# Tyler-Sch/pyruhvro

Measured on NVIDIA H100. Metric: avro_to_arrow_records_per_sec, higher is better.
Workload: dtype u8

## Files before the change

### include/ruhvro_b200.h

```cpp
#ifndef RUHVRO_B200_H
#define RUHVRO_B200_H

#include <stddef.h>
#include <stdint.h>

#ifdef __cplusplus
extern "C" {
#endif

struct ArrowSchema;
struct ArrowArray;
struct ArrowDeviceArray;

typedef struct rv_schema rv_schema;
typedef struct rv_result rv_result;
typedef struct rv_encoded rv_encoded;

typedef enum rv_status {
    RV_OK = 0,
    RV_ERR_EOF = 1,
    RV_ERR_VARINT = 2,
    RV_ERR_BOOL = 3,
    RV_ERR_NEG_LEN = 4,
    RV_ERR_BRANCH = 5,
    RV_ERR_ENUM = 6,
    RV_ERR_SCHEMA = 7,
    RV_ERR_OVERFLOW = 8,
    RV_ERR_INVALID = 9,
    RV_ERR_CUDA = 10,
    RV_ERR_VALUE = 11,
    RV_ERR_FRAME = 12
} rv_status;


rv_status rv_schema_parse(const char* json, size_t len, rv_schema** out);
rv_schema* rv_schema_retain(rv_schema* s);
void rv_schema_release(rv_schema* s);

int rv_schema_is_supported(const rv_schema* s);

rv_status rv_schema_export_arrow(const rv_schema* s, struct ArrowSchema* out);

rv_status rv_schema_project(const rv_schema* s, const char* const* columns, int64_t n_columns, rv_schema** out);


rv_status rv_decode_host(const rv_schema* s, const uint8_t* data, const int64_t* offsets, int64_t n,
                         int64_t num_chunks, rv_result** out);

rv_status rv_decode_device(const rv_schema* s, const uint8_t* d_data, const int64_t* d_offsets, int64_t n,
                           int64_t num_chunks, void* cuda_stream, rv_result** out);

typedef struct rv_framing {
    int32_t header_bytes;
    int32_t check_magic;
    int64_t schema_id;
} rv_framing;
rv_status rv_decode_host_framed(const rv_schema* s, const uint8_t* data, const int64_t* offsets, int64_t n,
                                int64_t num_chunks, const rv_framing* framing, rv_result** out);
rv_status rv_decode_device_framed(const rv_schema* s, const uint8_t* d_data, const int64_t* d_offsets, int64_t n,
                                  int64_t num_chunks, const rv_framing* framing, void* cuda_stream, rv_result** out);

rv_status rv_decode_ocf_host(const uint8_t* file, int64_t len, int64_t num_chunks, rv_schema** schema_out, rv_result** out);

rv_status rv_decode_ocf_host_projected(const uint8_t* file, int64_t len, int64_t num_chunks, const char* const* columns,
                                       int64_t n_columns, rv_schema** schema_out, rv_result** out);

rv_status rv_result_to_host(rv_result* r);

int64_t rv_result_num_batches(const rv_result* r);
int64_t rv_result_num_rows(const rv_result* r, int64_t batch);
int64_t rv_result_arrow_bytes(const rv_result* r);

int64_t rv_result_buffer_bytes(const rv_result* r);

rv_status rv_result_export(rv_result* r, int64_t batch, struct ArrowArray* out_array, struct ArrowSchema* out_schema);
rv_status rv_result_export_device(rv_result* r, int64_t batch, struct ArrowDeviceArray* out_array, struct ArrowSchema* out_schema);

void rv_result_free(rv_result* r);

rv_status rv_encode_host(const rv_schema* s, struct ArrowArray* batch, struct ArrowSchema* batch_schema, int64_t num_chunks, rv_encoded** out);
int64_t rv_encoded_num_chunks(const rv_encoded* r);
rv_status rv_encoded_export(rv_encoded* r, int64_t chunk, struct ArrowArray* out_array, struct ArrowSchema* out_schema);
void rv_encoded_free(rv_encoded* r);
int rv_last_encode_timings(float* out_ms, int cap);

typedef struct rv_gather rv_gather;
int64_t rv_gather_meta_len(const rv_schema* s);
rv_status rv_result_gather_meta(const rv_result* r, int64_t batch, int64_t* out, int64_t cap);
rv_status rv_gather_plan(const rv_schema* s, const int64_t* metas , int world, rv_gather** out);
int rv_gather_num_groups(const rv_gather* g);
int rv_gather_group_of_rank(const rv_gather* g, int rank);
rv_status rv_gather_group_info(const rv_gather* g, int group, int64_t* out5);
rv_status rv_gather_alloc(rv_gather* g, int group, void* cuda_stream, void** out_dev_ptr);
rv_status rv_gather_push(rv_gather* g, int group, int rank, rv_result* mine, int64_t batch, void* dst_base, void* cuda_stream);
rv_status rv_gather_finish(rv_gather* g, int group, rv_result** out);
void rv_gather_free(rv_gather* g);
rv_status rv_ipc_export(void* dev_ptr, uint8_t* handle64);
rv_status rv_ipc_open(const uint8_t* handle64, void** out_dev_ptr);
rv_status rv_ipc_close(void* dev_ptr);

rv_status rv_dev_rebase_i32(int32_t* d_dst, const int32_t* d_src, int64_t n, int32_t add, void* cuda_stream);
rv_status rv_dev_concat_bits(uint32_t* d_dst_words, int64_t dst_bit, const uint32_t* d_src_words, int64_t nbits, void* cuda_stream);


void* rv_host_alloc(size_t bytes);
void rv_host_free(void* p);

int rv_last_timings(float* out_ms, int cap);
int rv_last_launch_count(void);
int rv_last_passes(void);
void rv_schema_forget_stats(const rv_schema* s);

const char* rv_last_walker(void);
const char* rv_schema_jit_status(const rv_schema* s);
long long rv_last_slow_tiles(void);
void rv_set_jit_enabled(int enabled);

int64_t rv_schema_walker_source(const rv_schema* s, char* buf, size_t cap);

rv_status rv_schema_precompile(const rv_schema* s, const char* arch);

const char* rv_last_error(void);
const char* rv_version(void);

#ifdef __cplusplus
}
#endif

#endif
```

### pyruhvro_b200/__init__.py

```python
from __future__ import annotations

import ctypes
import os
import threading
from typing import List

import pyarrow as pa

from . import _build

__all__ = [
    "deserialize_array", "deserialize_array_threaded", "deserialize_array_threaded_spawn",
    "serialize_record_batch", "serialize_record_batch_spawn", "lib", "Schema", "decode_packed", "deserialize_arrow_array",
    "deserialize_confluent", "deserialize_ocf",
]

_HERE = os.path.dirname(os.path.abspath(__file__))


class _ArrowSchema(ctypes.Structure):
    _fields_ = [("format", ctypes.c_char_p), ("name", ctypes.c_char_p), ("metadata", ctypes.c_char_p),
                ("flags", ctypes.c_int64), ("n_children", ctypes.c_int64), ("children", ctypes.c_void_p),
                ("dictionary", ctypes.c_void_p), ("release", ctypes.c_void_p), ("private_data", ctypes.c_void_p)]


class _ArrowArray(ctypes.Structure):
    _fields_ = [("length", ctypes.c_int64), ("null_count", ctypes.c_int64), ("offset", ctypes.c_int64),
                ("n_buffers", ctypes.c_int64), ("n_children", ctypes.c_int64), ("buffers", ctypes.c_void_p),
                ("children", ctypes.c_void_p), ("dictionary", ctypes.c_void_p), ("release", ctypes.c_void_p),
                ("private_data", ctypes.c_void_p)]


def _load():
    path = os.path.join(_HERE, "libruhvro_b200.so")
    if os.environ.get("RV_LIB_PATH"):
        return _bind(ctypes.CDLL(os.environ["RV_LIB_PATH"]))
    try:
        _build.build_all()
    except Exception:
        if not os.path.exists(path):
            raise
    return _bind(ctypes.CDLL(path))


def _bind(L):
    vp, i64, cp = ctypes.c_void_p, ctypes.c_int64, ctypes.c_char_p
    L.rv_schema_parse.argtypes = [cp, ctypes.c_size_t, ctypes.POINTER(vp)]
    L.rv_schema_retain.restype = vp
    L.rv_schema_retain.argtypes = [vp]
    L.rv_schema_release.argtypes = [vp]
    L.rv_schema_release.restype = None
    L.rv_schema_is_supported.argtypes = [vp]
    L.rv_schema_export_arrow.argtypes = [vp, vp]
    L.rv_decode_host.argtypes = [vp, vp, vp, i64, i64, ctypes.POINTER(vp)]
    L.rv_decode_device.argtypes = [vp, vp, vp, i64, i64, vp, ctypes.POINTER(vp)]
    L.rv_decode_host_framed.argtypes = [vp, vp, vp, i64, i64, vp, ctypes.POINTER(vp)]
    L.rv_decode_device_framed.argtypes = [vp, vp, vp, i64, i64, vp, vp, ctypes.POINTER(vp)]
    L.rv_decode_ocf_host.argtypes = [vp, i64, i64, ctypes.POINTER(vp), ctypes.POINTER(vp)]
    L.rv_decode_ocf_host_projected.argtypes = [vp, i64, i64, vp, i64, ctypes.POINTER(vp), ctypes.POINTER(vp)]
    L.rv_schema_project.argtypes = [vp, vp, i64, ctypes.POINTER(vp)]
    L.rv_result_to_host.argtypes = [vp]
    L.rv_result_num_batches.restype = i64
    L.rv_result_num_batches.argtypes = [vp]
    L.rv_result_num_rows.restype = i64
    L.rv_result_num_rows.argtypes = [vp, i64]
    L.rv_result_arrow_bytes.restype = i64
    L.rv_result_arrow_bytes.argtypes = [vp]
    L.rv_result_buffer_bytes.restype = i64
    L.rv_result_buffer_bytes.argtypes = [vp]
    L.rv_result_export.argtypes = [vp, i64, vp, vp]
    L.rv_result_export_device.argtypes = [vp, i64, vp, vp]
    L.rv_result_free.argtypes = [vp]
    L.rv_result_free.restype = None
    L.rv_encode_host.argtypes = [vp, vp, vp, i64, ctypes.POINTER(vp)]
    L.rv_encoded_num_chunks.restype = i64
    L.rv_encoded_num_chunks.argtypes = [vp]
    L.rv_encoded_export.argtypes = [vp, i64, vp, vp]
    L.rv_encoded_free.argtypes = [vp]
    L.rv_encoded_free.restype = None
    L.rv_host_alloc.restype = vp
    L.rv_host_alloc.argtypes = [ctypes.c_size_t]
    L.rv_host_free.argtypes = [vp]
    L.rv_host_free.restype = None
    L.rv_last_timings.argtypes = [ctypes.POINTER(ctypes.c_float), ctypes.c_int]
    L.rv_last_launch_count.restype = ctypes.c_int
    L.rv_last_slow_tiles.restype = ctypes.c_longlong
    L.rv_last_passes.restype = ctypes.c_int
    L.rv_schema_forget_stats.argtypes = [vp]
    L.rv_schema_forget_stats.restype = None
    L.rv_last_walker.restype = cp
    L.rv_set_jit_enabled.argtypes = [ctypes.c_int]
    L.rv_set_jit_enabled.restype = None
    L.rv_schema_walker_source.restype = i64
    L.rv_schema_walker_source.argtypes = [vp, cp, ctypes.c_size_t]
    L.rv_schema_precompile.argtypes = [vp, cp]
    L.rv_last_error.restype = cp
    L.rv_version.restype = cp
    return L


lib = _load()


def last_walker() -> str:
    return (lib.rv_last_walker() or b"").decode()


def set_jit_enabled(enabled: int) -> None:
    lib.rv_set_jit_enabled(int(enabled))


def _last_error() -> str:
    return (lib.rv_last_error() or b"").decode("utf-8", "replace")


def _check(status: int):
    if status != 0:
        raise ValueError(_last_error())


class Schema:

    def __init__(self, schema_json: str):
        raw = schema_json.encode("utf-8")
        h = ctypes.c_void_p()
        _check(lib.rv_schema_parse(raw, len(raw), ctypes.byref(h)))
        self.handle = h.value
        self._arrow = None

    def __del__(self):
        h, self.handle = getattr(self, "handle", None), None
        if h:
            lib.rv_schema_release(h)

    @classmethod
    def _adopt(cls, handle: int) -> "Schema":
        s = cls.__new__(cls)
        s.handle, s._arrow = handle, None
        return s

    def project(self, columns) -> "Schema":
        names, keep = _column_names(columns)
        h = ctypes.c_void_p()
        _check(lib.rv_schema_project(self.handle, names, len(keep), ctypes.byref(h)))
        return Schema._adopt(h.value)

    @property
    def is_supported(self) -> bool:
        return bool(lib.rv_schema_is_supported(self.handle))

    def precompile(self, arch: str = "sm_90a") -> None:
        _check(lib.rv_schema_precompile(self.handle, arch.encode()))

    @property
    def walker_source(self) -> str:
        n = lib.rv_schema_walker_source(self.handle, None, 0)
        if n < 0:
            raise ValueError("schema has no decode plan")
        buf = ctypes.create_string_buffer(n + 1)
        lib.rv_schema_walker_source(self.handle, buf, n + 1)
        return buf.value.decode()

    @property
    def arrow_schema(self) -> pa.Schema:
        if self._arrow is None:
            cs = _ArrowSchema()
            _check(lib.rv_schema_export_arrow(self.handle, ctypes.addressof(cs)))
            self._arrow = pa.Schema._import_from_c(ctypes.addressof(cs))
        return self._arrow


def _column_names(columns):
    if isinstance(columns, (str, bytes)):
        raise TypeError("argument 'columns': expected a list of field names, not a single string")
    keep = []
    for c in columns:
        if not isinstance(c, str):
            raise TypeError("argument 'columns': field names must be str")
        keep.append(c.encode("utf-8"))
    arr = (ctypes.c_char_p * max(len(keep), 1))(*keep)
    return arr, keep


_schema_cache = {}
_schema_lock = threading.Lock()


def _get_or_parse_schema(schema: str, columns=None) -> Schema:
    if not isinstance(schema, str):
        raise TypeError("argument 'schema': expected str")
    if columns is not None:
        if isinstance(columns, (str, bytes)):
            raise TypeError("argument 'columns': expected a list of field names, not a single string")
        columns = tuple(columns)
    key = (schema, columns)
    with _schema_lock:
        s = _schema_cache.get(key)
    if s is not None:
        return s
    parsed = Schema(schema) if columns is None else _get_or_parse_schema(schema).project(columns)
    with _schema_lock:
        return _schema_cache.setdefault(key, parsed)


def _export_batches(result_handle: int, schema: Schema) -> List[pa.RecordBatch]:
    try:
        arrow_schema = schema.arrow_schema
        out = []
        for i in range(lib.rv_result_num_batches(result_handle)):
            arr = _ArrowArray()
            _check(lib.rv_result_export(result_handle, i, ctypes.addressof(arr), None))
            out.append(pa.RecordBatch._import_from_c(ctypes.addressof(arr), arrow_schema))
        return out
    finally:
        lib.rv_result_free(result_handle)


_native_mod = None


def _ext():
    global _native_mod
    if _native_mod is None:
        import importlib
        _native_mod = importlib.import_module(__name__ + "._native")
    return _native_mod


class Framing(ctypes.Structure):
    _fields_ = [("header_bytes", ctypes.c_int32), ("check_magic", ctypes.c_int32), ("schema_id", ctypes.c_int64)]


def _decode_list(records, schema: str, num_chunks: int, framing=None, columns=None) -> List[pa.RecordBatch]:
    if not isinstance(records, list):
        raise TypeError("argument 'list': expected a list of bytes")
    s = _get_or_parse_schema(schema, columns)
    if framing is None:
        handle = _ext().decode_list(s.handle, records, int(num_chunks))
    else:
        handle = _ext().decode_list(s.handle, records, int(num_chunks), *framing)
    return _export_batches(handle, s)




def deserialize_ocf(data, num_chunks=1, *, columns=None) -> List[pa.RecordBatch]:
    import numpy as np
    if num_chunks < 0:
        raise OverflowError("can't convert negative int to unsigned")
    buf = np.frombuffer(data, dtype=np.uint8)
    sh, h = ctypes.c_void_p(), ctypes.c_void_p()
    if columns is None:
        _check(lib.rv_decode_ocf_host(buf.ctypes.data if buf.size else None, buf.size, int(num_chunks), ctypes.byref(sh), ctypes.byref(h)))
    else:
        names, keep = _column_names(columns)
        _check(lib.rv_decode_ocf_host_projected(buf.ctypes.data if buf.size else None, buf.size, int(num_chunks), names, len(keep),
                                                ctypes.byref(sh), ctypes.byref(h)))
    return _export_batches(h.value, Schema._adopt(sh.value))


def deserialize_confluent(list, schema, num_chunks=1, schema_id=None, *, columns=None):
    if num_chunks < 0:
        raise OverflowError("can't convert negative int to unsigned")
    return _decode_list(list, schema, num_chunks, framing=(5, 1, -1 if schema_id is None else int(schema_id)), columns=columns)


def deserialize_array(list, schema, *, columns=None):
    return _decode_list(list, schema, 1, columns=columns)[0]


def deserialize_array_threaded(list, schema, num_chunks, *, columns=None):
    if num_chunks < 0:
        raise OverflowError("can't convert negative int to unsigned")
    return _decode_list(list, schema, num_chunks, columns=columns)


def deserialize_array_threaded_spawn(list, schema, num_chunks, *, columns=None):
    return deserialize_array_threaded(list, schema, num_chunks, columns=columns)


def decode_packed(data, offsets, n: int, schema: str, num_chunks: int = 1, framing: "Framing | None" = None, *,
                  columns=None) -> List[pa.RecordBatch]:
    import numpy as np
    s = _get_or_parse_schema(schema, columns)
    data = np.ascontiguousarray(data, dtype=np.uint8)
    offsets = np.ascontiguousarray(offsets, dtype=np.int64)
    h = ctypes.c_void_p()
    _check(lib.rv_decode_host_framed(s.handle, data.ctypes.data if data.size else None, offsets.ctypes.data, n, num_chunks,
                                     ctypes.byref(framing) if framing is not None else None, ctypes.byref(h)))
    return _export_batches(h.value, s)


def _packed_view(arr):
    import numpy as np
    if isinstance(arr, pa.ChunkedArray):
        arr = arr.combine_chunks() if arr.num_chunks != 1 else arr.chunk(0)
    t = arr.type
    if pa.types.is_large_binary(t) or pa.types.is_large_string(t):
        odt = np.int64
    elif pa.types.is_binary(t) or pa.types.is_string(t):
        odt = np.int32
    else:
        raise TypeError(f"expected a (Large)Binary / (Large)String array of Avro datums, got {t}")
    if arr.null_count:
        raise ValueError("the datum array contains nulls")
    n = len(arr)
    bufs = arr.buffers()
    if n == 0 or bufs[1] is None:
        return np.zeros(0, dtype=np.uint8), np.zeros(1, dtype=np.int64), 0
    off = np.frombuffer(bufs[1], dtype=odt)[arr.offset: arr.offset + n + 1]
    data = np.frombuffer(bufs[2], dtype=np.uint8) if bufs[2] is not None else np.zeros(0, dtype=np.uint8)
    return data, off.astype(np.int64, copy=False), n


def deserialize_arrow_array(array, schema, num_chunks=1, *, columns=None):
    if num_chunks < 0:
        raise OverflowError("can't convert negative int to unsigned")
    data, off, n = _packed_view(array)
    return decode_packed(data, off, n, schema, int(num_chunks), columns=columns)


def serialize_record_batch(data, schema, num_chunks):
    if not isinstance(data, pa.RecordBatch):
        raise TypeError("argument 'data': expected a pyarrow.RecordBatch")
    if num_chunks < 0:
        raise OverflowError("can't convert negative int to unsigned")
    s = _get_or_parse_schema(schema)
    c_arr, c_sch = _ArrowArray(), _ArrowSchema()
    data._export_to_c(ctypes.addressof(c_arr), ctypes.addressof(c_sch))
    h = ctypes.c_void_p()
    _check(lib.rv_encode_host(s.handle, ctypes.addressof(c_arr), ctypes.addressof(c_sch), int(num_chunks), ctypes.byref(h)))
    try:
        out = []
        for i in range(lib.rv_encoded_num_chunks(h)):
            a, sc = _ArrowArray(), _ArrowSchema()
            _check(lib.rv_encoded_export(h, i, ctypes.addressof(a), ctypes.addressof(sc)))
            out.append(pa.Array._import_from_c(ctypes.addressof(a), ctypes.addressof(sc)))
        return out
    finally:
        lib.rv_encoded_free(h)


def serialize_record_batch_spawn(data, schema, num_chunks):
    return serialize_record_batch(data, schema, num_chunks)
```

### pyruhvro_b200/csrc/dev_kernels.cuh

```cuda
#pragma once
#include "dev_core.cuh"

namespace rv {

struct Tile {
    int chunk;
    int local_tile;
    int lin;
    int64_t r0;
    int nrec;
    int64_t chunk_len;
};

__device__ __forceinline__ Tile tile_of(const DecodeParams& p, int id) {
    Tile t;
    int j = 0, local = id;
    if (p.k > 1) {
        const int body = p.k * p.tiles_per_chunk;
        if (id < body) {
            local = int(__fdividef(float(id), float(p.k)));
            while (local > 0 && local * p.k > id) --local;
            while ((local + 1) * p.k <= id) ++local;
            j = id - local * p.k;
        } else {
            j = p.k - 1;
            local = p.tiles_per_chunk + (id - body);
        }
    }
    t.chunk = j;
    t.local_tile = local;
    t.lin = j * p.tiles_per_chunk + local;
    const int64_t cs = int64_t(j) * p.chunk_rows;
    const int64_t ce = (j == p.k - 1) ? p.n : cs + p.chunk_rows;
    t.chunk_len = ce - cs;
    t.r0 = cs + int64_t(t.local_tile) * kBlock;
    const int64_t left = ce - t.r0;
    t.nrec = left < kBlock ? int(left) : kBlock;
    return t;
}

struct TileWindow {
    bool staged;
    bool tma;
    int64_t t0, t1;
    uint32_t mis;
    int64_t o0, o1;
    int64_t f0, f1;
};

__device__ __forceinline__ void l2_prefetch_line(const void* p) { asm volatile("prefetch.global.L2 [%0];" ::"l"(p)); }
__device__ __forceinline__ void l2_prefetch_bulk(const void* p, uint32_t bytes) {
    asm volatile("cp.async.bulk.prefetch.L2.global [%0], %1;" ::"l"(p), "r"(bytes) : "memory");
}
constexpr int kPrefetchLane = 32;

__device__ __forceinline__ uint32_t smem_addr(const void* p) { return uint32_t(__cvta_generic_to_shared(p)); }
__device__ __forceinline__ void mbar_init(uint32_t mbar, uint32_t arrivals) {
    asm volatile("mbarrier.init.shared::cta.b64 [%0], %1;" ::"r"(mbar), "r"(arrivals) : "memory");
    asm volatile("fence.mbarrier_init.release.cluster;" ::: "memory");
}
__device__ __forceinline__ void bulk_load(uint32_t dst, const void* src, uint32_t bytes, uint32_t mbar) {
    asm volatile("mbarrier.arrive.expect_tx.shared::cta.b64 _, [%0], %1;" ::"r"(mbar), "r"(bytes) : "memory");
    asm volatile("cp.async.bulk.shared::cluster.global.mbarrier::complete_tx::bytes [%0], [%1], %2, [%3];"
                 ::"r"(dst), "l"(src), "r"(bytes), "r"(mbar) : "memory");
}
__device__ __forceinline__ void mbar_wait(uint32_t mbar, uint32_t parity) {
    asm volatile(
        "{\n"
        ".reg .pred P1;\n"
        "RV_WAIT:\n"
        "mbarrier.try_wait.parity.shared::cta.b64 P1, [%0], %1;\n"
        "@P1 bra RV_DONE;\n"
        "bra RV_WAIT;\n"
        "RV_DONE:\n"
        "}" ::"r"(mbar), "r"(parity) : "memory");
}

constexpr unsigned long long kStAgg = 1ull << 62;
constexpr unsigned long long kStPrefix = 2ull << 62;
constexpr unsigned long long kStMask = (1ull << 62) - 1ull;

__device__ __forceinline__ unsigned long long ld_state(const unsigned long long* p) {
    unsigned long long v;
    asm volatile("ld.relaxed.gpu.global.u64 %0, [%1];" : "=l"(v) : "l"(p) : "memory");
    return v;
}
__device__ __forceinline__ void st_state(unsigned long long* p, unsigned long long v) {
    asm volatile("st.relaxed.gpu.global.u64 [%0], %1;" ::"l"(p), "l"(v) : "memory");
}

__device__ __forceinline__ unsigned long long look_back(const unsigned long long* st, const int tile, const int first) {
    const int lane = threadIdx.x & 31;
    unsigned long long excl = 0;
    int t = tile - 1;
    for (;;) {
        const int mine = t - lane;
        const bool real = mine >= first;
        unsigned long long v;
        do { v = real ? ld_state(st + mine) : kStPrefix; } while (__any_sync(0xFFFFFFFFu, (v >> 62) == 0ull));
        const unsigned has = __ballot_sync(0xFFFFFFFFu, (v >> 62) == 2ull);
        const int pl = has ? __ffs(int(has)) - 1 : 32;
        unsigned long long c = lane <= pl ? (v & kStMask) : 0ull;
#pragma unroll
        for (int d = 16; d; d >>= 1) c += __shfl_xor_sync(0xFFFFFFFFu, c, d);
        excl += c;
        if (has) break;
        t -= 32;
    }
    return excl;
}

template <class W>
__device__ __forceinline__ TileWindow stage_in(const DecodeParams& p, const Tile& t, const int tile_id, const SmemMap& m) {
    const int tid = threadIdx.x;
    if (tid == 0) mbar_init(smem_addr(rv_smem + m.mbar), 1);
    if (p.n_nodes) {
        uint4* dn = reinterpret_cast<uint4*>(rv_smem + m.nodes);
        for (int i = tid; i < p.n_nodes * 2; i += kBlock) dn[i] = __ldg(reinterpret_cast<const uint4*>(p.nodes) + i);
    }
    if (p.bufs) {
        void** sp = reinterpret_cast<void**>(rv_smem + m.ptrs);
        void* const* gp = p.bufs + size_t(t.chunk) * p.n_slots;
        for (int i = tid; i < p.n_slots; i += kBlock) sp[i] = gp[i];
    }
    if constexpr (!W::kRegCursors) {
        uint32_t* cur = reinterpret_cast<uint32_t*>(rv_smem + m.cur);
        for (int s = 0; s < p.n_streams; ++s) cur[s * kBlock + tid] = 0;
    }
    if (tid == 0) *reinterpret_cast<uint32_t*>(rv_smem + m.flags) = 0u;
    TileWindow w;
    w.t0 = __ldg(p.offsets + t.r0);
    w.t1 = __ldg(p.offsets + t.r0 + t.nrec);
    w.o0 = w.o1 = 0;
    if (tid < t.nrec) {
        w.o0 = __ldg(p.offsets + t.r0 + tid);
        w.o1 = __ldg(p.offsets + t.r0 + tid + 1);
    }
    w.f0 = w.f1 = -1;
    const int64_t ft = int64_t(tile_id) + p.prefetch_dist;
    if (p.prefetch_dist > 0 && ft < p.n_tiles) {
        const Tile f = tile_of(p, int(ft));
        if (tid < 17 && f.r0 + 16 * tid <= p.n) l2_prefetch_line(p.offsets + f.r0 + 16 * tid);
        if (tid == kPrefetchLane) {
            w.f0 = __ldg(p.offsets + f.r0);
            w.f1 = __ldg(p.offsets + f.r0 + f.nrec);
        }
    }
    const int64_t span = w.t1 - w.t0;
    w.mis = uint32_t(reinterpret_cast<uintptr_t>(p.data + w.t0) & 15u);
    w.staged = span >= 0 && uint64_t(span) + w.mis <= uint64_t(p.smem_data_cap);
    w.tma = false;
    if (w.staged) {
        const uint4* g = reinterpret_cast<const uint4*>(p.data + w.t0 - w.mis);
        const int nvec = int((span + w.mis + 15) >> 4);
        w.tma = nvec > 0;
        if (w.tma && tid == 0) bulk_load(smem_addr(rv_smem + m.in), g, uint32_t(nvec) << 4, smem_addr(rv_smem + m.mbar));
    }
    if (tid == 0) {
        if (span > 0 && static_cast<unsigned long long>(span) > p.ctrl[CW_MAX_SPAN]) atomicMax(p.ctrl + CW_MAX_SPAN, static_cast<unsigned long long>(span));
        if (t.lin == 0) p.ctrl[CW_IN_FIRST] = static_cast<unsigned long long>(w.t0);
        if (t.lin == p.n_tiles - 1) p.ctrl[CW_IN_LAST] = static_cast<unsigned long long>(w.t1);
    }
    return w;
}

__device__ __forceinline__ void wait_window(const TileWindow& w, const SmemMap& m) {
    if (w.tma) mbar_wait(smem_addr(rv_smem + m.mbar), 0);
}

template <class C>
__device__ __forceinline__ int64_t init_ctx(C& c, const DecodeParams& p, const Tile& t, const SmemMap& m, const TileWindow& w) {
    const int tid = threadIdx.x;
    const uint32_t s0 = smem_addr(rv_smem);
    c.nodes = reinterpret_cast<const DNode*>(rv_smem + m.nodes);
    c.cur = reinterpret_cast<uint32_t*>(rv_smem + m.cur) + tid;
    c.cur_stride = kBlock;
    c.sym_off = p.sym_off;
    c.sym_bytes = p.sym_bytes;
    c.bufs = p.bufs ? p.bufs + size_t(t.chunk) * p.n_slots : nullptr;
    c.ptrs_saddr = p.bufs ? s0 + m.ptrs : 0u;
    c.err = 0;
    c.pm = 0;
    c.usel = 0;
    c.stage_on = false;
    c.stage_saddr = s0 + m.stage;
    c.adj_saddr = s0 + m.adj;
    c.items_saddr = s0 + m.items;
    c.in_range = tid < t.nrec;
    c.row0 = uint32_t(t.local_tile) * kBlock + tid;
    c.store_word = (tid & 31) == 0 && int64_t(c.row0) < t.chunk_len;
    c.base = p.data;
    c.sbase = s0 + m.in;
    c.pos = c.end = 0;
    const int64_t r = t.r0 + tid;
    if (c.in_range) {
        const int64_t o0 = w.o0, o1 = w.o1;
        if (o1 < o0 || o1 - o0 > int64_t(0xFFFFFFF0u)) c.err = E_OVERFLOW;
        else if (C::kShared) {
            if (o0 < w.t0 || o1 > w.t1) c.err = E_OVERFLOW;
            else { c.pos = uint32_t(o0 - w.t0) + w.mis; c.end = uint32_t(o1 - w.t0) + w.mis; }
        } else {
            c.base = p.data + o0;
            c.end = uint32_t(o1 - o0);
        }
        if (p.frame_skip && !c.err) {
            if (c.end - c.pos < p.frame_skip) c.err = E_FRAME;
            else {
                if (p.frame_check) {
                    const uint32_t id = (ld_u8(c, c.pos + 1) << 24) | (ld_u8(c, c.pos + 2) << 16) | (ld_u8(c, c.pos + 3) << 8) | ld_u8(c, c.pos + 4);
                    if (ld_u8(c, c.pos) != 0u || (p.frame_check == 2 && id != p.frame_id)) c.err = E_FRAME;
                }
                c.pos += p.frame_skip;
            }
        }
    }
    return r;
}

__device__ __forceinline__ void report(const DecodeParams& p, int64_t record, uint32_t code) {
    atomicMin(p.ctrl + CW_ERR, (static_cast<unsigned long long>(record) << 8) | code);
}

__device__ __forceinline__ void prefetch_window(const DecodeParams& p, const TileWindow& w) {
    if (threadIdx.x == kPrefetchLane && w.f0 >= 0 && w.f1 > w.f0 && w.f1 - w.f0 < (int64_t(1) << 20)) {
        const uintptr_t a = reinterpret_cast<uintptr_t>(p.data + w.f0) & ~uintptr_t(15);
        const uintptr_t e = (reinterpret_cast<uintptr_t>(p.data + w.f1) + 15) & ~uintptr_t(15);
        l2_prefetch_bulk(reinterpret_cast<const void*>(a), uint32_t(e - a));
    }
}

template <class W, bool SM>
__device__ __forceinline__ uint32_t count_walk(const DecodeParams& p, const Tile& t, const SmemMap& m, const TileWindow& w, typename W::Cur& q) {
    WalkCtx<SM> c;
    const int64_t r = init_ctx(c, p, t, m, w);
    if constexpr (W::kRegCursors) {
#pragma unroll
        for (int s = 0; s < W::kStreams; ++s) q.v[s] = 0;
    } else {
        if (!SM) for (int s = 0; s < p.n_streams; ++s) c.cur[s * kBlock] = 0;
    }
#if !defined(RV_ABL_NOCOUNTWALK)
    W::template walk<WM_COUNT>(c, p.n_nodes, q);
#endif
    if (!SM && c.in_range && c.err) report(p, r, c.err);
    return c.in_range ? c.err : 0u;
}
template <class W>
struct CountOut { typename W::Cur q; uint32_t err; };
template <class W>
__device__ __noinline__ CountOut<W> count_walk_global(const DecodeParams p, const Tile t, const SmemMap m, const TileWindow w) {
    CountOut<W> o;
    o.err = count_walk<W, false>(p, t, m, w, o.q);
    return o;
}

__device__ __forceinline__ void stage_map(const DecodeParams& p, const Tile& t, const SmemMap& m) {
    const uint32_t* tbase = reinterpret_cast<const uint32_t*>(rv_smem + m.tbase);
    const uint32_t* ttot = reinterpret_cast<const uint32_t*>(rv_smem + m.ttot);
    uint32_t* adj = reinterpret_cast<uint32_t*>(rv_smem + m.adj);
    const int lane = threadIdx.x & 31;
    uint32_t carry = 0;
    for (int s0 = 0; s0 < p.n_streams; s0 += 32) {
        const int s = s0 + lane;
        uint32_t tb = 0, ga = 0, region = 0;
        int slot = -1;
        if (s < p.n_streams) {
            tb = tbase[s];
            slot = p.stream_slot[s];
            if (slot >= 0) {
                const uint8_t* b = *reinterpret_cast<uint8_t* const*>(rv_smem + m.ptrs + uint32_t(slot) * 8u);
                ga = uint32_t(reinterpret_cast<uintptr_t>(b + tb) & 15u);
                region = (ttot[s] + ga + 15u) & ~15u;
            }
        }
        uint32_t incl = region;
        for (int d = 1; d < 32; d <<= 1) {
            const uint32_t u = __shfl_up_sync(0xFFFFFFFFu, incl, d);
            if (lane >= d) incl += u;
        }
        if (s < p.n_streams) adj[s] = slot >= 0 ? (carry + incl - region + ga) - tb : 0u;
        carry += __shfl_sync(0xFFFFFFFFu, incl, 31);
    }
    if (lane == 0 && (p.n_utf8 == 0 || (p.smem_stage_cap > 0 && carry <= p.smem_stage_cap))) atomicOr(reinterpret_cast<uint32_t*>(rv_smem + m.flags), 2u);
    (void)t;
}

template <class W, bool SM>
__device__ __forceinline__ void emit_walk(const DecodeParams& p, const Tile& t, const SmemMap& m, const TileWindow& w, typename W::Cur& q, const bool stage_on) {
    WalkCtx<SM> c;
    (void)init_ctx(c, p, t, m, w);
    c.stage_on = stage_on;
    const int tid = threadIdx.x;
    if (t.local_tile == 0) {
        if (p.n_nodes) {
            for (int i = tid & 31; i < p.n_nodes; i += 32) {
                const DNode nd = c.nodes[i];
                if (nd.flags & NF_SKIP) continue;
                if (nd.kind == NK_STR || nd.kind == NK_ENUM || nd.kind == NK_LIST || nd.kind == NK_MAP || nd.kind == NK_BYTES)
                    static_cast<int32_t*>(buf_ptr(c, nd.slot_a))[0] = 0;
            }
        } else {
            W::zero_offsets(c, tid & 31);
        }
    }
#if !defined(RV_ABL_NOWALK)
    W::template walk<WM_EMIT>(c, p.n_nodes, q);
#endif
}
template <class W>
__device__ __noinline__ void emit_walk_global(const DecodeParams p, const Tile t, const SmemMap m, const TileWindow w, typename W::Cur q, const bool stage_on) {
    emit_walk<W, false>(p, t, m, w, q, stage_on);
}

__device__ __forceinline__ void stage_write_out(const DecodeParams& p, const SmemMap& m) {
    const uint32_t* tbase = reinterpret_cast<const uint32_t*>(rv_smem + m.tbase);
    const uint32_t* ttot = reinterpret_cast<const uint32_t*>(rv_smem + m.ttot);
    const uint32_t* adj = reinterpret_cast<const uint32_t*>(rv_smem + m.adj);
    const int warp = threadIdx.x >> 5, lane = threadIdx.x & 31;
    asm volatile("fence.proxy.async.shared::cta;" ::: "memory");
    __syncthreads();
    for (int s = warp; s < p.n_streams; s += kWarps) {
        const int slot = p.stream_slot[s];
        const uint32_t n = ttot[s];
        if (slot < 0 || n == 0) continue;
        const uint32_t tb = tbase[s];
        uint8_t* g = *reinterpret_cast<uint8_t* const*>(rv_smem + m.ptrs + uint32_t(slot) * 8u) + tb;
        const uint32_t so = m.stage + adj[s] + tb;
        const uint32_t head = min(n, (16u - uint32_t(reinterpret_cast<uintptr_t>(g) & 15u)) & 15u);
        for (uint32_t i = lane; i < head; i += 32) g[i] = rv_smem[so + i];
        const uint32_t nvec = (n - head) >> 4;
        if (lane == 0 && nvec > 0)
            asm volatile("cp.async.bulk.global.shared::cta.bulk_group [%0], [%1], %2;"
                         ::"l"(g + head), "r"(smem_addr(rv_smem + so + head)), "r"(nvec << 4) : "memory");
        const uint32_t done = head + (nvec << 4);
        for (uint32_t i = done + lane; i < n; i += 32) g[i] = rv_smem[so + i];
    }
    if (lane == 0) {
        asm volatile("cp.async.bulk.commit_group;" ::: "memory");
        asm volatile("cp.async.bulk.wait_group.read 0;" ::: "memory");
    }
}

template <class W>
__device__ __forceinline__ void fused_body(const DecodeParams& p, const int tile_id) {
    const Tile t = tile_of(p, tile_id);
    const SmemMap m = smem_map(p.n_nodes, p.n_streams, p.n_slots, p.smem_data_cap, p.smem_stage_cap, W::kRegCursors, W::kItemBytes);
    typename W::Cur q;
    const int tid = threadIdx.x, warp = tid >> 5, lane = tid & 31;
    const TileWindow w = stage_in<W>(p, t, tile_id, m);
    __syncthreads();
    wait_window(w, m);

    uint32_t my_err;
    bool warp_precise = false;
    if (w.staged) {
        my_err = count_walk<W, true>(p, t, m, w, q);
        const bool not_plain = my_err != 0u;
        if (not_plain) {
            const CountOut<W> o = count_walk_global<W>(p, t, m, w);
            q = o.q;
            my_err = o.err;
        }
        warp_precise = __any_sync(0xFFFFFFFFu, not_plain);
    } else {
        const CountOut<W> o = count_walk_global<W>(p, t, m, w);
        q = o.q;
        my_err = o.err;
    }

    constexpr int kPerLane = kBlock / 32;
    uint32_t* cur = reinterpret_cast<uint32_t*>(rv_smem + m.cur);
    uint32_t* ttot = reinterpret_cast<uint32_t*>(rv_smem + m.ttot);
    uint32_t* tbase = reinterpret_cast<uint32_t*>(rv_smem + m.tbase);
    uint32_t* flags = reinterpret_cast<uint32_t*>(rv_smem + m.flags);
    if constexpr (W::kRegCursors) {
#pragma unroll
        for (int s = 0; s < W::kStreams; ++s) cur[s * kBlock + tid] = q.v[s];
    }
    const bool any_err = __syncthreads_or(my_err != 0u) != 0;
    for (int s = warp; s < p.n_streams; s += kWarps) {
        uint32_t* cl = cur + s * kBlock + lane * kPerLane;
        uint32_t v[kPerLane];
        uint32_t any = 0;
        if constexpr (kPerLane % 4 == 0) {
#pragma unroll
            for (int i = 0; i < kPerLane; i += 4) {
                const uint4 x = *reinterpret_cast<const uint4*>(cl + i);
                v[i] = x.x; v[i + 1] = x.y; v[i + 2] = x.z; v[i + 3] = x.w;
                any |= x.x | x.y | x.z | x.w;
            }
        } else {
#pragma unroll
            for (int i = 0; i < kPerLane; ++i) { v[i] = cl[i]; any |= v[i]; }
        }
        uint32_t tile_total;
        if (__any_sync(0xFFFFFFFFu, any >= (0x80000000u / uint32_t(kBlock)))) {
            unsigned long long run = 0;
            if (lane == 0) {
                uint32_t* cs = cur + s * kBlock;
                for (int i = 0; i < kBlock; ++i) {
                    const uint32_t x = cs[i];
                    cs[i] = uint32_t(run);
                    run += x;
                }
                if (run > 0x7FFFFFFFull) { report(p, t.r0, E_OVERFLOW); run = 0x7FFFFFFFull; }
            }
            __syncwarp();
            tile_total = __shfl_sync(0xFFFFFFFFu, uint32_t(run), 0);
        } else {
            uint32_t tot = 0;
#pragma unroll
            for (int i = 0; i < kPerLane; ++i) {
                const uint32_t x = v[i];
                v[i] = tot;
                tot += x;
            }
            uint32_t incl = tot;
#pragma unroll
            for (int d = 1; d < 32; d <<= 1) {
                const uint32_t u = __shfl_up_sync(0xFFFFFFFFu, incl, d);
                if (lane >= d) incl += u;
            }
            const uint32_t base = incl - tot;
            if constexpr (kPerLane % 4 == 0) {
#pragma unroll
                for (int i = 0; i < kPerLane; i += 4)
                    *reinterpret_cast<uint4*>(cl + i) = make_uint4(base + v[i], base + v[i + 1], base + v[i + 2], base + v[i + 3]);
            } else {
#pragma unroll
                for (int i = 0; i < kPerLane; ++i) cl[i] = base + v[i];
            }
            tile_total = __shfl_sync(0xFFFFFFFFu, incl, 31);
        }
        if (lane == 0) {
            ttot[s] = tile_total;
            st_state(p.tile_state + size_t(s) * p.n_tiles + t.lin, (t.local_tile == 0 ? kStPrefix : kStAgg) | tile_total);
        }
    }
    __syncwarp();
    for (int s = warp; s < p.n_streams; s += kWarps) {
        unsigned long long base = 0;
        const uint32_t tot = ttot[s];
        if (t.local_tile != 0) {
            unsigned long long* st = p.tile_state + size_t(s) * p.n_tiles;
#if !defined(RV_ABL_NOLOOKBACK)
            base = look_back(st, t.lin, t.lin - t.local_tile);
#endif
            if (lane == 0) st_state(st + t.lin, kStPrefix | ((base + tot) & kStMask));
        }
        if (lane == 0) {
            const unsigned long long incl = base + tot;
            const bool last = int64_t(t.local_tile + 1) * kBlock >= t.chunk_len;
            if (last) {
                p.ctrl[CW_CHUNK_TOT + size_t(t.chunk) * p.n_streams + s] = incl;
                if (incl > 0x7FFFFFFFull) report(p, int64_t(t.chunk) * p.chunk_rows, E_OVERFLOW);
            }
            const unsigned long long cap = p.caps ? static_cast<unsigned long long>(p.caps[size_t(t.chunk) * p.n_streams + s]) : 0ull;
            if (incl > cap && !p.count_only) {
                atomicOr(flags, 1u);
                if (p.ctrl[CW_OVER] == 0ull) atomicMax(p.ctrl + CW_OVER, 1ull);
            }
            tbase[s] = uint32_t(base > 0x7FFFFFFFull ? 0x7FFFFFFFull : base);
        }
    }
    __syncthreads();
    if (warp == 0 && p.n_utf8 > 0) {
        uint32_t need = 0;
        for (int s = lane; s < p.n_streams; s += 32)
            if (p.stream_slot[s] >= 0) need += ttot[s] + 31u;
#pragma unroll
        for (int d = 16; d; d >>= 1) need += __shfl_xor_sync(0xFFFFFFFFu, need, d);
        if (lane == 0 && static_cast<unsigned long long>(need) > p.ctrl[CW_MAX_UTF8]) atomicMax(p.ctrl + CW_MAX_UTF8, static_cast<unsigned long long>(need));
    }
    if (p.count_only || any_err || (flags[0] & 1u)) return;

    if constexpr (W::kRegCursors) {
#pragma unroll
        for (int s = 0; s < W::kStreams; ++s) q.v[s] = cur[s * kBlock + tid] + tbase[s];
    } else {
        for (int s = 0; s < p.n_streams; ++s) cur[s * kBlock + tid] += tbase[s];
    }
    if constexpr (W::kRegCursors) __syncthreads();
    if (warp == 0) stage_map(p, t, m);
    if (w.staged && p.n_utf8 > 0) {
        uint4* z = reinterpret_cast<uint4*>(rv_smem + m.stage);
        for (uint32_t i = tid; i < (p.smem_stage_cap >> 4); i += kBlock) z[i] = make_uint4(0u, 0u, 0u, 0u);
    }
    __syncthreads();
    const bool fast = w.staged && (flags[0] & 2u);
    if (fast) {
        if (!warp_precise) emit_walk<W, true>(p, t, m, w, q, true);
        else emit_walk_global<W>(p, t, m, w, q, true);
        prefetch_window(p, w);
        if (p.n_utf8 > 0) stage_write_out(p, m);
    } else {
        if (tid == 0) atomicAdd(p.ctrl + CW_SLOW_TILES, 1ull);
        emit_walk_global<W>(p, t, m, w, q, false);
    }
}

}
```

### pyruhvro_b200/csrc/dev_types.h

```cpp
#pragma once

#if defined(__CUDACC_RTC__)
typedef signed char int8_t;
typedef unsigned char uint8_t;
typedef short int16_t;
typedef unsigned short uint16_t;
typedef int int32_t;
typedef unsigned int uint32_t;
typedef long long int64_t;
typedef unsigned long long uint64_t;
typedef unsigned long long uintptr_t;
typedef unsigned long size_t;
#else
#include <cstddef>
#include <cstdint>
#endif

namespace rv {

enum NodeKind : uint8_t {
    NK_I32 = 0,
    NK_I64 = 1,
    NK_F32 = 2,
    NK_F64 = 3,
    NK_BOOL = 4,
    NK_STR = 5,
    NK_ENUM = 6,
    NK_NULL = 7,
    NK_REC = 8,
    NK_UNION = 9,
    NK_LIST = 10,
    NK_MAP = 11,
    NK_BYTES = 12,
    NK_FIXED = 13,
    NK_DEC_BYTES = 14,
    NK_DEC_FIXED = 15,
    NK_UUID = 16
};

enum NodeFlags : uint8_t {
    NF_NULLABLE = 1,
    NF_NULL_FIRST = 2,
    NF_VALIDITY = 4,
    NF_ZERO_ITEMS = 8,
    NF_SKIP = 16
};

struct DNode {
    uint8_t kind;
    uint8_t flags;
    uint8_t level;
    uint8_t ulevel;
    uint8_t variant;
    uint8_t space;
    uint8_t pad0, pad1;
    int32_t end;
    int16_t slot_v;
    int16_t slot_a;
    int16_t slot_b;
    int16_t stream;
    int32_t aux;
    int32_t aux2;
    int32_t pad2;
};
static_assert(sizeof(DNode) == 32, "DNode layout is shared with the kernels");

constexpr int kMaxListDepth = 3;
constexpr int kMaxLevel = 31;
constexpr int kMaxUnionLevel = 8;
constexpr int kMaxStreams = 120;
constexpr int kMaxNodes = 1024;

enum ErrCode : uint32_t {
    E_OK = 0,
    E_EOF = 1,
    E_VARINT = 2,
    E_BOOL = 3,
    E_NEG_LEN = 4,
    E_BRANCH = 5,
    E_ENUM = 6,
    E_SCHEMA = 7,
    E_OVERFLOW = 8,
    E_FRAME = 12,
    E_VALUE = 11
};

#ifndef RV_KBLOCK
#define RV_KBLOCK 256
#endif
constexpr int kBlock = RV_KBLOCK;
static_assert(kBlock % 32 == 0 && kBlock >= 64 && kBlock <= 1024, "tiles are whole warps");
constexpr int kWarps = kBlock / 32;

enum CtrlWord : int {
    CW_ERR = 0,
    CW_MAX_SPAN = 1,
    CW_MAX_UTF8 = 2,
    CW_OVER = 3,
    CW_SLOW_TILES = 4,
    CW_IN_FIRST = 5,
    CW_IN_LAST = 6,
    CW_CHUNK_TOT = 8
};

struct DecodeParams {
    const uint8_t* data;
    const int64_t* offsets;
    int64_t n;
    int64_t chunk_rows;
    int32_t k;
    int32_t tiles_per_chunk;
    int32_t n_tiles;
    const DNode* nodes;
    int32_t n_nodes;
    int32_t n_streams;
    int32_t n_slots;
    const int32_t* sym_off;
    const uint8_t* sym_bytes;
    const int16_t* stream_slot;
    unsigned long long* tile_state;
    unsigned long long* ctrl;
    const uint32_t* caps;
    void* const* bufs;
    int32_t n_utf8;
    int32_t prefetch_dist;
    uint32_t smem_data_cap;
    uint32_t smem_stage_cap;
    int32_t count_only;
    uint32_t frame_skip;
    int32_t frame_check;
    uint32_t frame_id;
};

constexpr uint32_t kWindowPad = 64;

constexpr int kItemSlots = 4;
constexpr int kItemEntries = kItemSlots + 2;
constexpr uint32_t kItemSeq = 0xFFu;
#if defined(__CUDACC__)
__host__ __device__
#endif
constexpr uint32_t item_table_bytes(int n_lists) { return uint32_t(n_lists) * uint32_t(kItemEntries) * uint32_t(kBlock); }

struct SmemMap {
    uint32_t nodes, ttot, tbase, adj, flags, mbar, ptrs, items, cur, in, stage, total;
};

#if defined(__CUDACC__)
__host__ __device__
#endif
inline SmemMap smem_map(int n_nodes, int n_streams, int n_slots, uint32_t data_cap, uint32_t stage_cap, bool alias_cur, uint32_t item_bytes) {
    SmemMap m;
    m.nodes = 0;
    m.ttot = uint32_t(n_nodes) * 32u;
    m.tbase = m.ttot + uint32_t(n_streams + 1) * 4u;
    m.adj = m.tbase + uint32_t(n_streams) * 4u;
    m.flags = (m.adj + uint32_t(n_streams) * 4u + 15u) & ~15u;
    m.mbar = m.flags + 16u;
    m.ptrs = m.mbar + 16u;
    m.items = (m.ptrs + uint32_t(n_slots) * 8u + 15u) & ~15u;
    m.cur = (m.items + item_bytes + 15u) & ~15u;
    const uint32_t cur_bytes = uint32_t(n_streams) * kBlock * 4u;
    m.in = alias_cur ? m.cur : ((m.cur + cur_bytes + 15u) & ~15u);
    m.stage = (m.in + data_cap + kWindowPad + 15u) & ~15u;
    if (alias_cur) {
        m.cur = m.stage;
        m.total = m.stage + (stage_cap > cur_bytes ? stage_cap : cur_bytes);
    } else {
        m.total = m.stage + stage_cap;
    }
    return m;
}

}
```

### pyruhvro_b200/csrc/engine.cu

```cuda
#include <cuda_runtime.h>
#include <sched.h>
#include <sys/syscall.h>
#include <unistd.h>

#include <algorithm>
#include <atomic>
#include <chrono>
#include <condition_variable>
#include <cstdio>
#include <cstring>
#include <deque>
#include <functional>
#include <map>
#include <memory>
#include <mutex>
#include <stdexcept>
#include <string>
#include <thread>
#include <vector>

#include "../../include/ruhvro_b200.h"
#include "arrow_c.h"
#include "gather.hpp"
#include "ocf.hpp"
#include "jit.hpp"
#include "kernels.cuh"
#include "plan.hpp"
#include "result.hpp"
#include "schema.hpp"

using namespace rv;

namespace {

thread_local std::string t_error;
thread_local float t_timings[6] = {0, 0, 0, 0, 0, 0};
thread_local int t_launches = 0;
thread_local const char* t_walker = "none";
thread_local long long t_slow_tiles = 0;
thread_local int t_passes = 0;

double env_double(const char* name, double dflt) {
    const char* v = std::getenv(name);
    return v && *v ? std::atof(v) : dflt;
}

rv_status fail(rv_status st, const std::string& msg) {
    t_error = msg;
    return st;
}

#define RV_CUDA(expr)                                                                                  \
    do {                                                                                               \
        cudaError_t e_ = (expr);                                                                       \
        if (e_ != cudaSuccess)                                                                         \
            return fail(RV_ERR_CUDA, std::string(#expr) + ": " + cudaGetErrorString(e_));              \
    } while (0)

struct NumaInfo {
    int node = -1;
    cpu_set_t cpus;
    bool have_cpus = false;
};

bool numa_enabled() {
    static const bool on = [] { const char* e = std::getenv("RV_NUMA"); return !(e && e[0] == '0'); }();
    return on;
}

const NumaInfo& gpu_numa(int device) {
    static std::mutex mu;
    static std::map<int, NumaInfo> cache;
    std::lock_guard<std::mutex> g(mu);
    auto it = cache.find(device);
    if (it != cache.end()) return it->second;
    NumaInfo info;
    CPU_ZERO(&info.cpus);
    char bus[64] = {0};
    if (numa_enabled() && cudaDeviceGetPCIBusId(bus, int(sizeof bus) - 1, device) == cudaSuccess) {
        for (char* c = bus; *c; ++c) *c = char(std::tolower(static_cast<unsigned char>(*c)));
        const std::string path = std::string("/sys/bus/pci/devices/") + bus + "/numa_node";
        if (FILE* f = std::fopen(path.c_str(), "r")) {
            int node = -1;
            if (std::fscanf(f, "%d", &node) == 1) info.node = node;
            std::fclose(f);
        }
        if (info.node >= 0) {
            const std::string cl = "/sys/devices/system/node/node" + std::to_string(info.node) + "/cpulist";
            if (FILE* f = std::fopen(cl.c_str(), "r")) {
                char buf[4096] = {0};
                if (std::fgets(buf, sizeof buf, f)) {
                    const char* c = buf;
                    while (*c) {
                        char* e = nullptr;
                        long a = std::strtol(c, &e, 10);
                        if (e == c) break;
                        long b = a;
                        if (*e == '-') { c = e + 1; b = std::strtol(c, &e, 10); }
                        for (long x = a; x <= b && x < CPU_SETSIZE; ++x) { CPU_SET(int(x), &info.cpus); info.have_cpus = true; }
                        c = (*e == ',') ? e + 1 : e;
                        if (*e != ',') break;
                    }
                }
                std::fclose(f);
            }
        }
    } else {
        (void)cudaGetLastError();
    }
    return cache[device] = info;
}

void prefer_node(int node) {
#if defined(SYS_set_mempolicy)
    if (node < 0) { (void)syscall(SYS_set_mempolicy, 0 , nullptr, 0UL); return; }
    unsigned long mask[16] = {0};
    if (node >= int(sizeof mask * 8)) return;
    mask[node / (8 * sizeof(unsigned long))] |= 1UL << (node % (8 * sizeof(unsigned long)));
    (void)syscall(SYS_set_mempolicy, 1 , mask, (unsigned long)(sizeof mask * 8 + 1));
#else
    (void)node;
#endif
}

void bind_thread_to_gpu_node(int device) {
    const NumaInfo& ni = gpu_numa(device);
    if (ni.node < 0) return;
    if (ni.have_cpus) {
        cpu_set_t cur, both;
        CPU_ZERO(&cur);
        if (sched_getaffinity(0, sizeof cur, &cur) == 0) {
            CPU_AND(&both, &cur, &ni.cpus);
            if (CPU_COUNT(&both) > 0) (void)sched_setaffinity(0, sizeof both, &both);
        }
    }
    prefer_node(ni.node);
}

class PinnedCache {
  public:
    void* get(size_t bytes, size_t* actual) {
        size_t want = round(bytes);
        {
            std::lock_guard<std::mutex> g(mu_);
            auto it = free_.lower_bound(want);
            if (it != free_.end() && it->first <= want + want / 4 + (1u << 20)) {
                void* p = it->second;
                *actual = it->first;
                cached_ -= it->first;
                free_.erase(it);
                return p;
            }
        }
        int device = 0, node = -1;
        if (cudaGetDevice(&device) == cudaSuccess) node = gpu_numa(device).node; else (void)cudaGetLastError();
        if (node >= 0) prefer_node(node);
        void* p = nullptr;
        if (cudaHostAlloc(&p, want, cudaHostAllocDefault) != cudaSuccess) {
            (void)cudaGetLastError();
            trim(0);
            if (cudaHostAlloc(&p, want, cudaHostAllocDefault) != cudaSuccess) { (void)cudaGetLastError(); p = nullptr; }
        }
        if (node >= 0) prefer_node(-1);
        if (!p) return nullptr;
        *actual = want;
        return p;
    }
    void put(void* p, size_t actual) {
        if (!p) return;
        {
            std::lock_guard<std::mutex> g(mu_);
            if (cached_ + actual <= kMaxCached) {
                free_.emplace(actual, p);
                cached_ += actual;
                return;
            }
        }
        cudaFreeHost(p);
    }
    void trim(size_t keep) {
        std::lock_guard<std::mutex> g(mu_);
        while (cached_ > keep && !free_.empty()) {
            auto it = std::prev(free_.end());
            cudaFreeHost(it->second);
            cached_ -= it->first;
            free_.erase(it);
        }
    }

  private:
    static constexpr size_t kMaxCached = size_t(24) << 30;
    static size_t round(size_t b) {
        size_t g = b >= (size_t(64) << 20) ? (size_t(16) << 20) : (b >= (1u << 20) ? (1u << 20) : 65536);
        return ((b ? b : 1) + g - 1) / g * g;
    }
    std::mutex mu_;
    std::multimap<size_t, void*> free_;
    size_t cached_ = 0;
};

class DeviceCache {
  public:
    void* get(size_t bytes, int device, size_t* actual) {
        const size_t want = round(bytes);
        {
            std::lock_guard<std::mutex> g(mu_);
            auto& fl = free_[device];
            auto it = fl.lower_bound(want);
            if (it != fl.end() && it->first <= want + want / 4 + (size_t(1) << 20)) {
                void* p = it->second;
                *actual = it->first;
                cached_ -= it->first;
                fl.erase(it);
                return p;
            }
        }
        void* p = nullptr;
        if (cudaMalloc(&p, want) != cudaSuccess) {
            (void)cudaGetLastError();
            trim(device);
            if (cudaMalloc(&p, want) != cudaSuccess) { (void)cudaGetLastError(); return nullptr; }
        }
        *actual = want;
        return p;
    }
    void put(void* p, size_t actual, int device) {
        if (!p) return;
        {
            std::lock_guard<std::mutex> g(mu_);
            if (cached_ + actual <= kMaxCached) {
                free_[device].emplace(actual, p);
                cached_ += actual;
                return;
            }
        }
        cudaFree(p);
    }
    void trim(int device) {
        std::lock_guard<std::mutex> g(mu_);
        auto& fl = free_[device];
        for (auto& kv : fl) { cudaFree(kv.second); cached_ -= kv.first; }
        fl.clear();
    }

  private:
    static constexpr size_t kMaxCached = size_t(40) << 30;
    static size_t round(size_t b) {
        const size_t g = b >= (size_t(32) << 20) ? (size_t(4) << 20) : (b >= (size_t(1) << 20) ? (size_t(256) << 10) : 4096);
        return ((b ? b : 1) + g - 1) / g * g;
    }
    std::mutex mu_;
    std::map<int, std::multimap<size_t, void*>> free_;
    size_t cached_ = 0;
};

DeviceCache& devmem() {
    static DeviceCache* c = new DeviceCache();
    return *c;
}

cudaStream_t worker_stream(int device, int w) {
    static std::mutex mu;
    static std::map<std::pair<int, int>, cudaStream_t> streams;
    std::lock_guard<std::mutex> g(mu);
    auto key = std::make_pair(device, w);
    auto it = streams.find(key);
    if (it != streams.end()) return it->second;
    cudaStream_t s = nullptr;
    if (cudaStreamCreateWithFlags(&s, cudaStreamNonBlocking) != cudaSuccess) s = nullptr;
    streams[key] = s;
    return s;
}

std::mutex g_host_mu;
std::map<void*, size_t> g_host_sizes;

PinnedCache& pinned() {
    static PinnedCache* c = new PinnedCache();
    return *c;
}

rv_status ensure_cuda(int* device) {
    static std::mutex mu;
    static std::vector<char> inited;
    int n = 0;
    cudaError_t e = cudaGetDeviceCount(&n);
    if (e != cudaSuccess || n == 0)
        return fail(RV_ERR_CUDA, std::string("no CUDA device available (this library has no CPU fallback): ") + cudaGetErrorString(e));
    RV_CUDA(cudaGetDevice(device));
    std::lock_guard<std::mutex> g(mu);
    if (inited.size() < size_t(n)) inited.resize(size_t(n), 0);
    if (!inited[size_t(*device)]) {
        RV_CUDA(prepare_kernels());
        cudaMemPool_t pool;
        RV_CUDA(cudaDeviceGetDefaultMemPool(&pool, *device));
        unsigned long long thr = ~0ull;
        RV_CUDA(cudaMemPoolSetAttribute(pool, cudaMemPoolAttrReleaseThreshold, &thr));
        inited[size_t(*device)] = 1;
    }
    return RV_OK;
}

struct DevBuf {
    void* p = nullptr;
    size_t actual = 0;
    int device = 0;
    cudaError_t alloc(size_t bytes, cudaStream_t) {
        if (cudaGetDevice(&device) != cudaSuccess) return cudaErrorInvalidDevice;
        p = devmem().get(bytes, device, &actual);
        return p ? cudaSuccess : cudaErrorMemoryAllocation;
    }
    ~DevBuf() { if (p) devmem().put(p, actual, device); }
};

}

struct DevicePlan {
    DNode* nodes = nullptr;
    int32_t* sym_off = nullptr;
    uint8_t* sym_bytes = nullptr;
    int16_t* stream_slot = nullptr;
};

struct JitState {
    bool tried = false;
    bool ok = false;
    std::string status = "not compiled";
    cudaLibrary_t lib = nullptr;
    cudaKernel_t fused = nullptr;
};

struct SchemaStats {
    bool valid = false;
    std::vector<double> per_row;
    double in_per_row = 0;
    unsigned long long max_span = 0;
    unsigned long long max_utf8 = 0;
};

struct rv_schema {
    std::atomic<int> refs{1};
    std::shared_ptr<const AvroNode> avro;
    bool supported = false;
    std::string why;
    std::vector<ArrowField> fields;
    bool has_fields = false;
    std::vector<int> keep;
    Plan plan;
    bool has_plan = false;
    std::mutex mu;
    std::map<int, DevicePlan> dev;
    std::map<int, JitState> jit;
    SchemaStats stats;
};

namespace {

rv_status device_plan(rv_schema* s, int device, DevicePlan* out) {
    std::lock_guard<std::mutex> g(s->mu);
    auto it = s->dev.find(device);
    if (it != s->dev.end()) { *out = it->second; return RV_OK; }
    DevicePlan d;
    const Plan& p = s->plan;
    RV_CUDA(cudaMalloc(&d.nodes, std::max<size_t>(1, p.nodes.size()) * sizeof(DNode)));
    RV_CUDA(cudaMalloc(&d.sym_off, std::max<size_t>(1, p.sym_off.size()) * 4));
    RV_CUDA(cudaMalloc(&d.sym_bytes, std::max<size_t>(1, p.sym_bytes.size())));
    std::vector<int16_t> sslot(std::max<size_t>(1, p.streams.size()), int16_t(-1));
    for (size_t i = 0; i < p.streams.size(); ++i)
        if (!p.streams[i].is_rows) sslot[i] = p.nodes[size_t(p.streams[i].node)].slot_b;
    RV_CUDA(cudaMalloc(&d.stream_slot, sslot.size() * 2));
    RV_CUDA(cudaMemcpy(d.stream_slot, sslot.data(), sslot.size() * 2, cudaMemcpyHostToDevice));
    RV_CUDA(cudaMemcpy(d.nodes, p.nodes.data(), p.nodes.size() * sizeof(DNode), cudaMemcpyHostToDevice));
    if (!p.sym_off.empty()) RV_CUDA(cudaMemcpy(d.sym_off, p.sym_off.data(), p.sym_off.size() * 4, cudaMemcpyHostToDevice));
    if (!p.sym_bytes.empty()) RV_CUDA(cudaMemcpy(d.sym_bytes, p.sym_bytes.data(), p.sym_bytes.size(), cudaMemcpyHostToDevice));
    s->dev[device] = d;
    *out = d;
    return RV_OK;
}

std::atomic<int> g_jit_override{-1};

bool jit_enabled() {
    const int o = g_jit_override.load(std::memory_order_relaxed);
    if (o >= 0) return o != 0;
    const char* e = std::getenv("RV_JIT");
    return !(e && e[0] == '0');
}

std::string device_arch(int device) {
    if (const char* e = std::getenv("RV_JIT_ARCH")) return e;
    cudaDeviceProp prop;
    if (cudaGetDeviceProperties(&prop, device) != cudaSuccess) return "sm_90a";
    return "sm_" + std::to_string(prop.major) + std::to_string(prop.minor) + ((prop.major >= 9) ? "a" : "");
}

JitState ensure_jit(rv_schema* s, int device) {
    if (!jit_enabled()) { JitState d; d.tried = true; d.status = "disabled (RV_JIT=0 / rv_set_jit_enabled(0))"; return d; }
    std::lock_guard<std::mutex> g(s->mu);
    JitState& j = s->jit[device];
    if (j.tried) return j;
    j.tried = true;
    const std::string source = generate_kernel_source(s->plan), arch = device_arch(device);
    for (int attempt = 0; attempt < 2; ++attempt) {
        std::vector<char> cubin;
        std::string log;
        if (!jit_cubin(source, arch, &cubin, &log, attempt > 0)) { j.status = "NVRTC: " + log; return j; }
        cudaError_t e = cudaLibraryLoadData(&j.lib, cubin.data(), nullptr, nullptr, 0, nullptr, nullptr, 0);
        if (e == cudaSuccess) e = cudaLibraryGetKernel(&j.fused, j.lib, "rvj_fused");
        if (e == cudaSuccess) e = cudaFuncSetAttribute(reinterpret_cast<const void*>(j.fused), cudaFuncAttributeMaxDynamicSharedMemorySize, 227 * 1024);
        if (e == cudaSuccess) e = cudaFuncSetAttribute(reinterpret_cast<const void*>(j.fused), cudaFuncAttributePreferredSharedMemoryCarveout, 100);
        if (e == cudaSuccess) { j.ok = true; j.status = "ok"; return j; }
        j.status = std::string("loading the compiled walker failed: ") + cudaGetErrorString(e);
        (void)cudaGetLastError();
        if (j.lib) { cudaLibraryUnload(j.lib); j.lib = nullptr; }
        j.fused = nullptr;
    }
    return j;
}

}

namespace {

struct Arena {
    void* dev = nullptr;
    size_t dev_actual = 0;
    size_t bytes = 0;
    void* host = nullptr;
    size_t host_actual = 0;
    size_t host_bytes = 0;
    int device = 0;
    void drop_device() {
        if (dev) devmem().put(dev, dev_actual, device);
        dev = nullptr;
    }
    ~Arena() {
        drop_device();
        if (host) pinned().put(host, host_actual);
    }
};

}

struct rv_result {
    rv_schema* schema = nullptr;
    std::vector<ChunkOut> chunks;
    std::vector<std::shared_ptr<Arena>> arenas;
    int64_t arrow_bytes = 0;
    ~rv_result() { if (schema) rv_schema_release(schema); }
};

namespace {

const char* err_text(uint32_t code) {
    switch (code) {
        case E_EOF: return "unexpected end of buffer";
        case E_VARINT: return "zigzag varint too long";
        case E_BOOL: return "invalid boolean byte";
        case E_NEG_LEN: return "negative string length";
        case E_BRANCH: return "invalid union branch index";
        case E_ENUM: return "enum index out of range";
        case E_OVERFLOW: return "Arrow i32 offset overflow (or malformed input offsets)";
        case E_VALUE: return "value does not fit its logical type (uuid text / decimal wider than 128 bits)";
        case E_FRAME: return "framed message: shorter than its header, wrong magic byte or unexpected schema id";
        default: return "decode error";
    }
}

struct HostScratch {
    uint8_t* p = nullptr;
    size_t cap = 0;
    ~HostScratch() { if (p) { cudaFreeHost(p); (void)cudaGetLastError(); } }
    uint8_t* get(size_t bytes) {
        if (bytes > cap) {
            if (p) cudaFreeHost(p);
            p = nullptr;
            cap = 0;
            const size_t want = std::max<size_t>(bytes * 2, 1 << 16);
            if (cudaHostAlloc(reinterpret_cast<void**>(&p), want, cudaHostAllocDefault) != cudaSuccess) { (void)cudaGetLastError(); p = nullptr; return nullptr; }
            cap = want;
        }
        return p;
    }
};
thread_local HostScratch t_scratch;

struct EventPool {
    cudaEvent_t ev[8] = {};
    int device = -1;
    ~EventPool() { for (auto& e : ev) if (e) cudaEventDestroy(e); (void)cudaGetLastError(); }
    cudaError_t get(int dev, cudaEvent_t** out) {
        if (device != dev) {
            for (auto& e : ev) { if (e) cudaEventDestroy(e); e = nullptr; }
            for (auto& e : ev) { const cudaError_t r = cudaEventCreate(&e); if (r != cudaSuccess) return r; }
            device = dev;
        }
        *out = ev;
        return cudaSuccess;
    }
};
thread_local EventPool t_events;

size_t align_up(size_t v, size_t a) { return (v + a - 1) / a * a; }

struct StageRing {
    static constexpr size_t kPiece = size_t(8) << 20;
    uint8_t* buf[2] = {nullptr, nullptr};
    cudaEvent_t done[2] = {nullptr, nullptr};
    int device = -1;
    ~StageRing() { release(); }
    void release() {
        for (int i = 0; i < 2; ++i) {
            if (buf[i]) cudaFreeHost(buf[i]);
            if (done[i]) cudaEventDestroy(done[i]);
            buf[i] = nullptr; done[i] = nullptr;
        }
        (void)cudaGetLastError();
        device = -1;
    }
    bool ready(int dev) {
        if (device == dev) return true;
        release();
        for (int i = 0; i < 2; ++i) {
            if (cudaHostAlloc(reinterpret_cast<void**>(&buf[i]), kPiece, cudaHostAllocDefault) != cudaSuccess ||
                cudaEventCreateWithFlags(&done[i], cudaEventDisableTiming) != cudaSuccess) { release(); return false; }
        }
        device = dev;
        return true;
    }
    cudaError_t upload(uint8_t* dst, const uint8_t* src, size_t bytes, cudaStream_t stream) {
        int slot = 0;
        for (size_t o = 0; o < bytes; o += kPiece, slot ^= 1) {
            const size_t len = std::min(kPiece, bytes - o);
            cudaError_t e = cudaEventSynchronize(done[slot]);
            if (e != cudaSuccess) return e;
            std::memcpy(buf[slot], src + o, len);
            e = cudaMemcpyAsync(dst + o, buf[slot], len, cudaMemcpyHostToDevice, stream);
            if (e == cudaSuccess) e = cudaEventRecord(done[slot], stream);
            if (e != cudaSuccess) return e;
        }
        return cudaSuccess;
    }
};
thread_local StageRing t_stage;

bool is_pageable(const void* p) {
    cudaPointerAttributes at{};
    if (cudaPointerGetAttributes(&at, p) != cudaSuccess) { (void)cudaGetLastError(); return true; }
    return at.type == cudaMemoryTypeUnregistered;
}

cudaError_t upload(uint8_t* dst, const uint8_t* src, size_t bytes, int device, cudaStream_t stream) {
    if (bytes >= (size_t(1) << 20) && is_pageable(src) && t_stage.ready(device)) return t_stage.upload(dst, src, bytes, stream);
    return cudaMemcpyAsync(dst, src, bytes, cudaMemcpyHostToDevice, stream);
}


struct SyncOnExit {
    cudaStream_t stream;
    bool armed = true;
    ~SyncOnExit() { if (armed) { cudaStreamSynchronize(stream); (void)cudaGetLastError(); } }
};

struct InputHints {
    int64_t total_bytes = -1;
    int64_t max_span = -1;
    rv_framing framing = {0, 0, -1};
};

rv_status decode_on_device(rv_schema* s, const uint8_t* d_data, const int64_t* d_offsets, int64_t n, int64_t num_chunks,
                           const InputHints& hints, cudaStream_t stream, int device, rv_result** out, int64_t record_base = 0) {
    const Plan& plan = s->plan;
    const int S = int(plan.streams.size());
    const int Sx = std::max(S, 1);
    const int n_slots = int(plan.slots.size());
    int64_t k64 = clamp_chunks(num_chunks, n);
    if (k64 > (int64_t(1) << 24)) return fail(RV_ERR_INVALID, "num_chunks above 2^24 is not supported");
    const int k = int(k64);
    const int64_t chunk_rows = n / k;
    const int64_t last_rows = n - chunk_rows * (k - 1);

    auto res = std::make_unique<rv_result>();
    res->schema = rv_schema_retain(s);
    auto arena_sp = std::make_shared<Arena>();
    arena_sp->device = device;

    for (int i = 0; i < 4; ++i) t_timings[i] = 0;
    t_launches = 0;
    t_passes = 0;
    static const bool trace = std::getenv("RV_TRACE") && std::getenv("RV_TRACE")[0] == '1';
    auto t_prev = std::chrono::steady_clock::now();
    std::string trace_line;
    auto mark = [&](const char* what) {
        if (!trace) return;
        const auto now = std::chrono::steady_clock::now();
        trace_line += std::string(what) + "=" + std::to_string(std::chrono::duration<double, std::micro>(now - t_prev).count()).substr(0, 6) + "us ";
        t_prev = now;
    };

    std::vector<unsigned long long> chunk_tot(size_t(k) * size_t(Sx), 0ull);

    if (n == 0) {
        Layout L = compute_layout(plan, 0, k, chunk_tot.data());
        res->chunks = std::move(L.chunks);
        arena_sp->bytes = L.total_bytes;
        arena_sp->dev = devmem().get(std::max<size_t>(L.total_bytes, 64), device, &arena_sp->dev_actual);
        if (!arena_sp->dev) return fail(RV_ERR_CUDA, "device allocation of the Arrow buffer arena failed");
        res->arenas.assign(res->chunks.size(), arena_sp);
        RV_CUDA(cudaMemsetAsync(arena_sp->dev, 0, std::max<size_t>(L.total_bytes, 64), stream));
        RV_CUDA(cudaStreamSynchronize(stream));
        res->arrow_bytes = exported_bytes(plan, res->chunks);
        *out = res.release();
        return RV_OK;
    }

    DevicePlan dp;
    rv_status st = device_plan(s, device, &dp);
    if (st) return st;
    const int64_t tpc = std::max<int64_t>(1, (chunk_rows + kBlock - 1) / kBlock);
    const int64_t tiles_last = (last_rows + kBlock - 1) / kBlock;
    const int64_t n_tiles = tpc * (k - 1) + tiles_last;
    if (n_tiles > 0x7FFFFFF0ll) return fail(RV_ERR_INVALID, "too many records for one call");

    const JitState jit = ensure_jit(s, device);
    const bool use_jit = jit.ok;
    t_walker = use_jit ? "jit" : "interp";
    const int plan_nodes = use_jit ? 0 : int(plan.nodes.size());

    SchemaStats stats;
    {
        std::lock_guard<std::mutex> g(s->mu);
        stats = s->stats;
    }

    DecodeParams p{};
    p.data = d_data; p.offsets = d_offsets; p.n = n; p.chunk_rows = chunk_rows; p.k = k;
    p.tiles_per_chunk = int32_t(tpc); p.n_tiles = int32_t(n_tiles);
    p.nodes = dp.nodes; p.n_nodes = int32_t(plan_nodes); p.n_streams = S; p.n_slots = n_slots;
    p.sym_off = dp.sym_off; p.sym_bytes = dp.sym_bytes; p.stream_slot = dp.stream_slot;
    p.n_utf8 = 0;
    for (int i = 0; i < S; ++i) p.n_utf8 += plan.streams[size_t(i)].is_rows ? 0 : 1;
    p.frame_skip = uint32_t(std::max(hints.framing.header_bytes, 0));
    p.frame_check = hints.framing.check_magic ? (hints.framing.schema_id >= 0 ? 2 : 1) : 0;
    p.frame_id = uint32_t(hints.framing.schema_id >= 0 ? hints.framing.schema_id : 0);

    const size_t limit = 227 * 1024;
    const size_t cur_bytes = size_t(S) * kBlock * 4;
    const uint32_t item_bytes = use_jit ? item_table_bytes(item_parallel_lists(plan)) : 0u;
    const size_t fixed = smem_map(plan_nodes, S, n_slots, 0, 0, use_jit, item_bytes).stage;
    if (fixed + (use_jit ? cur_bytes : 0) + 2048 > limit) return fail(RV_ERR_SCHEMA, "schema too wide for the shared-memory cursor table");
    size_t smem_bytes = 0;
    auto configure = [&](const SchemaStats& st_) {
        const double in_per_row = hints.total_bytes >= 0 ? double(hints.total_bytes) / double(n) : (st_.in_per_row > 0 ? st_.in_per_row : 128.0);
        unsigned long long max_span = hints.max_span >= 0 ? static_cast<unsigned long long>(hints.max_span)
                                      : (st_.max_span ? st_.max_span + st_.max_span / 16 : static_cast<unsigned long long>(in_per_row * kBlock * 1.25));
        size_t want_in = std::min<size_t>(size_t(max_span), size_t(in_per_row * kBlock * env_double("RV_IN_CLAMP", 1.5))) + 48;
        want_in = std::max<size_t>(align_up(want_in, 64), 2048);
        const size_t room = (limit - fixed - 64) & ~size_t(15);
        const size_t min_stage = use_jit ? align_up(cur_bytes, 16) : 0;
        size_t cap_in = std::min(want_in, room - std::min(room, min_stage));
        size_t cap_stage = 0;
        if (p.n_utf8 > 0) {
            const size_t seen = st_.max_utf8 ? size_t(st_.max_utf8 + st_.max_utf8 / 16) : cap_in + size_t(p.n_utf8) * 31;
            double utf8_per_row = 0;
            if (st_.valid) for (int i = 0; i < S; ++i) if (!plan.streams[size_t(i)].is_rows) utf8_per_row += st_.per_row[size_t(i)];
            size_t want_out = seen;
            if (st_.valid) want_out = std::min<size_t>(seen, size_t(utf8_per_row * kBlock * env_double("RV_OUT_CLAMP", 1.5)) + size_t(p.n_utf8) * 31);
            cap_stage = align_up(want_out + 64, 64);
            if (const char* ev_ = std::getenv("RV_NO_STAGE_OUT")) if (ev_[0] == '1') cap_stage = 0;
        }
        cap_stage = std::max(cap_stage, min_stage);
        if (cap_in + cap_stage > room) cap_stage = std::max<size_t>(min_stage, (room - cap_in) & ~size_t(15));
        if (hints.max_span < 0 && (st_.max_span || st_.max_utf8)) {
            auto ctas = [&](size_t in_b, size_t st_b) { return (228 * 1024) / (smem_map(plan_nodes, S, n_slots, uint32_t(in_b), uint32_t(st_b), use_jit, item_bytes).total + 1024); };
            const size_t floor_in = st_.max_span ? std::min(cap_in, std::max<size_t>(align_up(size_t(st_.max_span) + 48, 64), 2048)) : cap_in;
            const size_t floor_stage = st_.max_utf8 ? std::min(cap_stage, std::max(min_stage, size_t(align_up(size_t(st_.max_utf8) + 64, 64)))) : cap_stage;
            const size_t want = ctas(cap_in, cap_stage) + 1;
            size_t in_b = cap_in, st_b = cap_stage;
            while (ctas(in_b, st_b) < want && (in_b > floor_in || st_b > floor_stage)) {
                if (in_b - floor_in >= st_b - floor_stage) in_b = std::max(floor_in, in_b - 64);
                else st_b = std::max(floor_stage, st_b - 64);
            }
            if (ctas(in_b, st_b) >= want) { cap_in = in_b; cap_stage = st_b; }
        }
        p.smem_data_cap = uint32_t(cap_in);
        p.smem_stage_cap = uint32_t(cap_stage);
        const size_t pad_smem = size_t(env_double("RV_SMEM_PAD", 0));
        smem_bytes = std::min<size_t>(smem_map(plan_nodes, S, n_slots, p.smem_data_cap, p.smem_stage_cap, use_jit, item_bytes).total + pad_smem, limit);
        p.prefetch_dist = 0;
        if (!(std::getenv("RV_NO_PREFETCH") && std::getenv("RV_NO_PREFETCH")[0] == '1')) {
            const int ctas_per_sm = int(std::max<size_t>(1, std::min<size_t>(8, (228 * 1024) / (smem_bytes + 1024))));
            int sms = 132;
            cudaDeviceGetAttribute(&sms, cudaDevAttrMultiProcessorCount, device);
            p.prefetch_dist = sms * ctas_per_sm;
        }
    };

    const int nv = int(plan.validity_slots.size());
    const size_t ctrl_words = size_t(CW_CHUNK_TOT) + chunk_tot.size();
    const size_t off_ctrl = 0;
    const size_t off_ones = align_up(off_ctrl + ctrl_words * 8, 16);
    const size_t ones_n = size_t(k) * size_t(std::max(nv, 1));
    const size_t back_bytes = off_ones + ones_n * 8;
    const size_t off_bufs = align_up(back_bytes, 16);
    const size_t off_caps = align_up(off_bufs + size_t(k) * size_t(n_slots) * sizeof(void*), 16);
    const size_t off_jobs = align_up(off_caps + size_t(k) * size_t(Sx) * 4, 16);
    const size_t misc_bytes = align_up(off_jobs + size_t(k) * size_t(std::max(nv, 1)) * sizeof(NullCountJob), 16);
    uint8_t* h_misc = t_scratch.get(misc_bytes + back_bytes);
    if (!h_misc) return fail(RV_ERR_CUDA, "pinned allocation of the call state failed");
    uint8_t* h_back = h_misc + misc_bytes;
    DevBuf d_misc, d_state;
    RV_CUDA(d_misc.alloc(misc_bytes, stream));
    RV_CUDA(d_state.alloc(size_t(Sx) * size_t(n_tiles) * 8, stream));
    SyncOnExit guard{stream};
    uint8_t* dm = static_cast<uint8_t*>(d_misc.p);
    p.ctrl = reinterpret_cast<unsigned long long*>(dm + off_ctrl);
    p.tile_state = static_cast<unsigned long long*>(d_state.p);
    cudaEvent_t* ev = nullptr;
    RV_CUDA(t_events.get(device, &ev));
    mark("setup");

    auto rows_of = [&](int j) { return j == k - 1 ? last_rows : chunk_rows; };
    std::vector<unsigned long long> caps(chunk_tot.size(), 0ull);
    bool exact_caps = false;
    bool count_only = !stats.valid;
    if (stats.valid) {
        const double margin = env_double("RV_CAP_MARGIN", 1.10);
        const double in_bytes = hints.total_bytes >= 0 ? double(hints.total_bytes) : double(n) * stats.in_per_row * 2.0 + 65536.0;
        double planned = 0;
        for (int j = 0; j < k; ++j)
            for (int i = 0; i < S; ++i) {
                double want = double(rows_of(j)) * stats.per_row[size_t(i)] * margin + 4096.0;
                const Stream& st_ = plan.streams[size_t(i)];
                const bool enum_text = !st_.is_rows && plan.nodes[size_t(st_.node)].kind == NK_ENUM;
                if (!enum_text) want = std::min(want, in_bytes + 4096.0);
                caps[size_t(j) * size_t(Sx) + size_t(i)] = static_cast<unsigned long long>(std::min(want, 2147483647.0));
                planned += want;
            }
        if (planned > 64.0 * in_bytes + double(size_t(1) << 30)) count_only = true;
    }
    Layout capL;
    std::vector<long long> ones(ones_n, 0);
    unsigned long long* hb_ctrl = reinterpret_cast<unsigned long long*>(h_back + off_ctrl);

    for (int pass = 0; pass < 3; ++pass) {
        ++t_passes;
        configure(stats);
        if (trace)
            trace_line += "smem=" + std::to_string(smem_bytes) + "(in " + std::to_string(p.smem_data_cap) + " stage " + std::to_string(p.smem_stage_cap) +
                          " items " + std::to_string(item_bytes) + "; largest tile seen: span " + std::to_string(stats.max_span) +
                          " utf8 " + std::to_string(stats.max_utf8) + ") ";
        uint8_t* arena = nullptr;
        if (!count_only) {
            capL = compute_layout(plan, n, k, caps.data());
            arena_sp->drop_device();
            arena_sp->bytes = capL.total_bytes;
            arena_sp->dev = devmem().get(std::max<size_t>(capL.total_bytes, 64), device, &arena_sp->dev_actual);
            if (!arena_sp->dev) {
                if (!exact_caps) { count_only = true; }
                else return fail(RV_ERR_CUDA, "device allocation of the Arrow buffer arena failed (" + std::to_string(capL.total_bytes) + " bytes)");
            } else {
                arena = static_cast<uint8_t*>(arena_sp->dev);
            }
        }
        std::memset(h_misc, 0, misc_bytes);
        unsigned long long* hc = reinterpret_cast<unsigned long long*>(h_misc + off_ctrl);
        hc[CW_ERR] = ~0ull;
        hc[CW_MAX_SPAN] = stats.max_span;
        hc[CW_MAX_UTF8] = stats.max_utf8;
        if (!count_only) {
            void** hb = reinterpret_cast<void**>(h_misc + off_bufs);
            for (int j = 0; j < k; ++j)
                for (int sl = 0; sl < n_slots; ++sl) hb[size_t(j) * size_t(n_slots) + size_t(sl)] = arena + capL.chunks[size_t(j)].slot_off[size_t(sl)];
            uint32_t* hcap = reinterpret_cast<uint32_t*>(h_misc + off_caps);
            for (size_t i = 0; i < caps.size(); ++i) hcap[i] = uint32_t(caps[i]);
            NullCountJob* jobs = reinterpret_cast<NullCountJob*>(h_misc + off_jobs);
            for (int j = 0; j < k; ++j)
                for (int v = 0; v < nv; ++v) {
                    const int sl = plan.validity_slots[size_t(v)];
                    const int space = plan.slots[size_t(sl)].space;
                    NullCountJob& job = jobs[size_t(j) * size_t(nv) + size_t(v)];
                    job.bitmap = reinterpret_cast<const uint32_t*>(arena + capL.chunks[size_t(j)].slot_off[size_t(sl)]);
                    job.n_bits = rows_of(j);
                    job.n_bits_dev = space == 0 ? nullptr : p.ctrl + CW_CHUNK_TOT + size_t(j) * size_t(Sx) + size_t(plan.space_stream[size_t(space)]);
                }
        }
        p.bufs = count_only ? nullptr : reinterpret_cast<void* const*>(dm + off_bufs);
        p.caps = count_only ? nullptr : reinterpret_cast<const uint32_t*>(dm + off_caps);
        p.count_only = count_only ? 1 : 0;

        RV_CUDA(cudaMemcpyAsync(dm, h_misc, misc_bytes, cudaMemcpyHostToDevice, stream));
        RV_CUDA(cudaMemsetAsync(d_state.p, 0, size_t(Sx) * size_t(n_tiles) * 8, stream));
        if (!count_only && capL.zero_bytes) RV_CUDA(cudaMemsetAsync(arena, 0, capL.zero_bytes, stream));
        RV_CUDA(cudaEventRecord(ev[0], stream));
        if (use_jit) {
            void* args[] = {&p};
            const cudaError_t le = cudaLaunchKernel(reinterpret_cast<const void*>(jit.fused), dim3(unsigned(p.n_tiles)), dim3(kBlock), args, smem_bytes, stream);
            if (le != cudaSuccess) {
                (void)cudaGetLastError();
                {
                    std::lock_guard<std::mutex> g(s->mu);
                    JitState& j = s->jit[device];
                    j.ok = false;
                    j.status = std::string("launch of the compiled walker was rejected: ") + cudaGetErrorString(le);
                }
                RV_CUDA(cudaStreamSynchronize(stream));
                return decode_on_device(s, d_data, d_offsets, n, num_chunks, hints, stream, device, out, record_base);
            }
        } else {
            launch_fused(p, smem_bytes, stream);
        }
        RV_CUDA(cudaEventRecord(ev[1], stream));
        t_launches += 1;
        if (!count_only && nv > 0) {
            launch_null_count(reinterpret_cast<const NullCountJob*>(dm + off_jobs), k * nv, reinterpret_cast<long long*>(dm + off_ones), stream);
            t_launches += 1;
        }
        RV_CUDA(cudaEventRecord(ev[2], stream));
        RV_CUDA(cudaGetLastError());
        RV_CUDA(cudaMemcpyAsync(h_back, dm, back_bytes, cudaMemcpyDeviceToHost, stream));
        mark("launched");
        RV_CUDA(cudaStreamSynchronize(stream));
        mark("sync");

        const unsigned long long err_word = hb_ctrl[CW_ERR];
        if (err_word != ~0ull) {
            const uint32_t code = uint32_t(err_word & 0xFF);
            return fail(rv_status(code), std::string(err_text(code)) + " (record " + std::to_string(int64_t(err_word >> 8) + record_base) + ")");
        }
        std::memcpy(chunk_tot.data(), hb_ctrl + CW_CHUNK_TOT, chunk_tot.size() * 8);
        const bool over = hb_ctrl[CW_OVER] != 0ull;
        t_slow_tiles = (long long)hb_ctrl[CW_SLOW_TILES];
        float ms = 0;
        cudaEventElapsedTime(&ms, ev[0], ev[1]);
        {
            std::lock_guard<std::mutex> g(s->mu);
            SchemaStats& ss = s->stats;
            if (ss.per_row.size() != size_t(S)) ss.per_row.assign(size_t(S), 0.0);
            for (int i = 0; i < S; ++i) {
                double worst = 0;
                for (int j = 0; j < k; ++j) worst = std::max(worst, double(chunk_tot[size_t(j) * size_t(Sx) + size_t(i)]) / double(std::max<int64_t>(rows_of(j), 1)));
                double& r = ss.per_row[size_t(i)];
                r = (!ss.valid || worst > r) ? worst : r * 0.9 + worst * 0.1;
            }
            if (hints.total_bytes >= 0) ss.in_per_row = double(hints.total_bytes) / double(n);
            else if (hb_ctrl[CW_IN_LAST] >= hb_ctrl[CW_IN_FIRST]) ss.in_per_row = double(hb_ctrl[CW_IN_LAST] - hb_ctrl[CW_IN_FIRST]) / double(n);
            ss.max_span = std::max(ss.max_span, hb_ctrl[CW_MAX_SPAN]);
            ss.max_utf8 = std::max(ss.max_utf8, hb_ctrl[CW_MAX_UTF8]);
            ss.valid = true;
            stats = ss;
        }
        if (!count_only && !over) {
            t_timings[0] = ms;
            cudaEventElapsedTime(&t_timings[3], ev[1], ev[2]);
            std::memcpy(ones.data(), h_back + off_ones, ones_n * 8);
            break;
        }
        t_timings[1] += ms;
        if (exact_caps) return fail(RV_ERR_CUDA, "internal error: exact-size pass reported a capacity overflow");
        caps = chunk_tot;
        exact_caps = true;
        count_only = false;
    }

    Layout L = compute_layout(plan, n, k, chunk_tot.data());
    for (int j = 0; j < k; ++j) L.chunks[size_t(j)].slot_off = capL.chunks[size_t(j)].slot_off;
    res->chunks = std::move(L.chunks);
    res->arenas.assign(res->chunks.size(), arena_sp);
    for (int j = 0; j < k; ++j)
        for (int v = 0; v < nv; ++v) {
            const int sl = plan.validity_slots[size_t(v)];
            ChunkOut& c = res->chunks[size_t(j)];
            c.null_count[size_t(sl)] = c.space_rows[size_t(plan.slots[size_t(sl)].space)] - ones[size_t(j) * size_t(nv) + size_t(v)];
        }
    res->arrow_bytes = exported_bytes(plan, res->chunks);
    mark("finish");
    if (trace) std::fprintf(stderr, "[rv trace] passes=%d %s\n", t_passes, trace_line.c_str());
    guard.armed = false;
    *out = res.release();
    return RV_OK;
}

rv_status check_decodable(const rv_schema* s) {
    if (!s) return fail(RV_ERR_INVALID, "null schema handle");
    if (!s->supported)
        return fail(RV_ERR_SCHEMA, "schema is outside the direct-decode subset (" + s->why + "); this library has no Value-tree CPU fallback");
    if (!s->has_plan) return fail(RV_ERR_SCHEMA, s->why);
    return RV_OK;
}

}

extern "C" {

rv_status rv_schema_parse(const char* json, size_t len, rv_schema** out) {
    if (!json || !out) return fail(RV_ERR_INVALID, "null argument");
    *out = nullptr;
    try {
        auto s = std::make_unique<rv_schema>();
        s->avro = parse_avro_schema(json, len);
        s->supported = is_supported(*s->avro, &s->why);
        if (s->avro->k == AK::Record) {
            try {
                s->fields = to_arrow_fields(*s->avro);
                s->has_fields = true;
            } catch (const std::exception& e) {
                if (s->supported) { s->supported = false; s->why = e.what(); }
            }
        }
        if (s->supported && s->has_fields) {
            try {
                s->plan = build_plan(*s->avro, s->fields);
                s->has_plan = true;
            } catch (const std::exception& e) {
                s->why = e.what();
            }
        }
        *out = s.release();
        return RV_OK;
    } catch (const std::exception& e) {
        return fail(RV_ERR_SCHEMA, e.what());
    }
}

rv_schema* rv_schema_retain(rv_schema* s) {
    if (s) s->refs.fetch_add(1, std::memory_order_relaxed);
    return s;
}

void rv_schema_release(rv_schema* s) {
    if (!s) return;
    if (s->refs.fetch_sub(1, std::memory_order_acq_rel) == 1) {
        for (auto& kv : s->dev) {
            cudaFree(kv.second.nodes);
            cudaFree(kv.second.sym_off);
            cudaFree(kv.second.sym_bytes);
            cudaFree(kv.second.stream_slot);
        }
        for (auto& kv : s->jit)
            if (kv.second.lib) cudaLibraryUnload(kv.second.lib);
        (void)cudaGetLastError();
        delete s;
    }
}

int rv_schema_is_supported(const rv_schema* s) { return s && s->supported && s->has_plan ? 1 : 0; }

rv_status rv_schema_project(const rv_schema* s, const char* const* columns, int64_t n_columns, rv_schema** out) {
    if (!s || !out || (!columns && n_columns != 0) || n_columns < 0) return fail(RV_ERR_INVALID, "null argument");
    *out = nullptr;
    rv_status st = check_decodable(s);
    if (st) return st;
    std::vector<std::string> names, requested;
    for (const ArrowField& f : s->fields) names.push_back(f.name);
    for (int64_t i = 0; i < n_columns; ++i) {
        if (!columns[i]) return fail(RV_ERR_INVALID, "column projection: null column name");
        requested.emplace_back(columns[i]);
    }
    try {
        const std::vector<int> sel = select_columns(names, requested);
        auto p = std::make_unique<rv_schema>();
        p->avro = s->avro;
        p->supported = true;
        p->has_fields = true;
        std::vector<ArrowField> all = s->keep.empty() ? s->fields : to_arrow_fields(*s->avro);
        for (int i : sel) {
            p->keep.push_back(s->keep.empty() ? i : s->keep[size_t(i)]);
            p->fields.push_back(s->fields[size_t(i)]);
        }
        p->plan = build_plan(*p->avro, all, &p->keep);
        p->has_plan = true;
        *out = p.release();
        return RV_OK;
    } catch (const std::invalid_argument& e) {
        return fail(RV_ERR_INVALID, e.what());
    } catch (const std::exception& e) {
        return fail(RV_ERR_SCHEMA, e.what());
    }
}

rv_status rv_schema_export_arrow(const rv_schema* s, struct ArrowSchema* out) {
    if (!s || !out) return fail(RV_ERR_INVALID, "null argument");
    if (!s->has_fields) return fail(RV_ERR_SCHEMA, s->why.empty() ? "top-level schema is not a record" : s->why);
    try {
        export_arrow_schema(s->fields, out);
        return RV_OK;
    } catch (const std::exception& e) {
        return fail(RV_ERR_SCHEMA, e.what());
    }
}

static rv_status framing_ok(const rv_framing* f) {
    if (!f) return RV_OK;
    if (f->header_bytes < 0 || f->header_bytes > 4096) return fail(RV_ERR_INVALID, "framing: header_bytes out of range");
    if (f->check_magic && f->header_bytes < 5) return fail(RV_ERR_INVALID, "framing: the Confluent header check needs header_bytes >= 5");
    if (f->schema_id > int64_t(0xFFFFFFFFu)) return fail(RV_ERR_INVALID, "framing: schema_id is a u32");
    return RV_OK;
}

rv_status rv_decode_device_framed(const rv_schema* s, const uint8_t* d_data, const int64_t* d_offsets, int64_t n,
                                  int64_t num_chunks, const rv_framing* framing, void* cuda_stream, rv_result** out) {
    if (!out) return fail(RV_ERR_INVALID, "null argument");
    *out = nullptr;
    rv_status st = check_decodable(s);
    if (st) return st;
    st = framing_ok(framing);
    if (st) return st;
    if (n < 0 || (n > 0 && (!d_data || !d_offsets))) return fail(RV_ERR_INVALID, "bad input pointers");
    if (reinterpret_cast<uintptr_t>(d_data) & 15u) return fail(RV_ERR_INVALID, "d_data must be 16-byte aligned");
    int device = 0;
    st = ensure_cuda(&device);
    if (st) return st;
    cudaStream_t stream = static_cast<cudaStream_t>(cuda_stream);
    InputHints hints;
    if (framing) hints.framing = *framing;
    try {
        st = decode_on_device(const_cast<rv_schema*>(s), d_data, d_offsets, n, num_chunks, hints, stream, device, out);
    } catch (const std::exception& e) {
        st = fail(RV_ERR_INVALID, e.what());
    }
    if (st) { const std::string keep = t_error; cudaStreamSynchronize(stream); (void)cudaGetLastError(); t_error = keep; }
    return st;
}

rv_status rv_decode_device(const rv_schema* s, const uint8_t* d_data, const int64_t* d_offsets, int64_t n,
                           int64_t num_chunks, void* cuda_stream, rv_result** out) {
    return rv_decode_device_framed(s, d_data, d_offsets, n, num_chunks, nullptr, cuda_stream, out);
}

}

namespace {

rv_status arena_to_host(rv_result& r, Arena& a, cudaStream_t stream, float* ms) {
    if (a.host) return RV_OK;
    const Plan& plan = r.schema->plan;
    const int n_slots = int(plan.slots.size());
    std::vector<size_t> mine;
    for (size_t i = 0; i < r.chunks.size(); ++i)
        if (r.arenas[i].get() == &a) mine.push_back(i);
    size_t total = 0;
    std::vector<CompactJob> jobs;
    std::vector<std::vector<size_t>> new_off(mine.size(), std::vector<size_t>(size_t(n_slots), 0));
    const uint8_t* src = static_cast<const uint8_t*>(a.dev);
    for (int pass = 0; pass < 2; ++pass)
        for (size_t mi = 0; mi < mine.size(); ++mi) {
            const ChunkOut& c = r.chunks[mine[mi]];
            for (int sl = 0; sl < n_slots; ++sl) {
                const Slot& slot = plan.slots[size_t(sl)];
                if (slot.zero_init != (pass == 0)) continue;
                size_t bytes = size_t(c.slot_bytes[size_t(sl)]);
                if (slot.role == SlotRole::Validity || slot.role == SlotRole::Bits) bytes = size_t((c.space_rows[size_t(slot.space)] + 31) / 32) * 4;
                new_off[mi][size_t(sl)] = total;
                if (bytes) jobs.push_back(CompactJob{src + c.slot_off[size_t(sl)], reinterpret_cast<uint8_t*>(total), int64_t(bytes)});
                total += (std::max<size_t>(bytes, 1) + 63) & ~size_t(63);
            }
        }
    const size_t host_bytes = std::max<size_t>(total, 64);
    size_t actual = 0;
    void* h = pinned().get(host_bytes, &actual);
    if (!h) return fail(RV_ERR_CUDA, "pinned host allocation failed");
    DevBuf packed, d_jobs;
    cudaError_t e = packed.alloc(host_bytes, stream);
    if (e == cudaSuccess) e = d_jobs.alloc(std::max<size_t>(jobs.size(), 1) * sizeof(CompactJob), stream);
    uint8_t* h_jobs = t_scratch.get(std::max<size_t>(jobs.size(), 1) * sizeof(CompactJob));
    if (e != cudaSuccess || !h_jobs) { pinned().put(h, actual); return fail(RV_ERR_CUDA, "device allocation for the host export failed"); }
    SyncOnExit guard{stream};
    for (CompactJob& job : jobs) job.dst = static_cast<uint8_t*>(packed.p) + reinterpret_cast<size_t>(job.dst);
    std::memcpy(h_jobs, jobs.data(), jobs.size() * sizeof(CompactJob));
    cudaEvent_t* ev = nullptr;
    e = t_events.get(a.device, &ev);
    if (e == cudaSuccess && !jobs.empty()) e = cudaMemcpyAsync(d_jobs.p, h_jobs, jobs.size() * sizeof(CompactJob), cudaMemcpyHostToDevice, stream);
    if (e == cudaSuccess && !jobs.empty()) {
        const int parts = int(std::max<size_t>(1, std::min<size_t>(64, (total / std::max<size_t>(jobs.size(), 1)) >> 16)));
        launch_compact(static_cast<const CompactJob*>(d_jobs.p), int(jobs.size()), parts, stream);
        e = cudaGetLastError();
    }
    if (e == cudaSuccess) e = cudaEventRecord(ev[6], stream);
    if (e == cudaSuccess) e = cudaMemcpyAsync(h, packed.p, host_bytes, cudaMemcpyDeviceToHost, stream);
    if (e == cudaSuccess) e = cudaEventRecord(ev[7], stream);
    if (e == cudaSuccess) e = cudaStreamSynchronize(stream);
    if (e != cudaSuccess) {
        (void)cudaStreamSynchronize(stream);
        (void)cudaGetLastError();
        pinned().put(h, actual);
        return fail(RV_ERR_CUDA, std::string("device->host copy: ") + cudaGetErrorString(e));
    }
    float t = 0;
    cudaEventElapsedTime(&t, ev[6], ev[7]);
    if (ms) *ms += t;
    guard.armed = false;
    a.host = h;
    a.host_actual = actual;
    a.host_bytes = host_bytes;
    a.drop_device();
    for (size_t mi = 0; mi < mine.size(); ++mi) r.chunks[mine[mi]].slot_off = new_off[mi];
    return RV_OK;
}

rv_status decode_host_range(rv_schema* s, const uint8_t* data, const int64_t* offsets, int64_t r0, int64_t r1, int64_t num_chunks,
                            cudaStream_t stream, int device, rv_result** out, float* h2d_ms, float* d2h_ms, const rv_framing& framing) {
    const int64_t n = r1 - r0;
    DevBuf d_data, d_off;
    InputHints hints;
    hints.framing = framing;
    const uint8_t* base = nullptr;
    rv_status st = RV_OK;
    if (n > 0) {
        const int64_t b0 = offsets[r0];
        const int64_t total = offsets[r1] - b0;
        if (total < 0) return fail(RV_ERR_INVALID, "offsets are not monotonic");
        hints.total_bytes = total;
        {
            const int64_t k = clamp_chunks(num_chunks, n);
            const int64_t cr = n / k;
            int64_t mx = 0;
            for (int64_t j = 0; j < k; ++j) {
                const int64_t cs = r0 + j * cr, ce = (j == k - 1) ? r1 : cs + cr;
                for (int64_t a = cs; a < ce; a += kBlock) mx = std::max(mx, offsets[std::min(a + kBlock, ce)] - offsets[a]);
            }
            hints.max_span = mx;
        }
        RV_CUDA(d_data.alloc(size_t(total) + 64, stream));
        RV_CUDA(d_off.alloc(size_t(n + 1) * 8, stream));
        cudaEvent_t* ev = nullptr;
        RV_CUDA(t_events.get(device, &ev));
        cudaEventRecord(ev[4], stream);
        cudaError_t e = upload(static_cast<uint8_t*>(d_data.p) + (b0 & 15), data + b0, size_t(total), device, stream);
        if (e == cudaSuccess) e = upload(static_cast<uint8_t*>(d_off.p), reinterpret_cast<const uint8_t*>(offsets + r0), size_t(n + 1) * 8, device, stream);
        cudaEventRecord(ev[5], stream);
        if (e != cudaSuccess) { (void)cudaStreamSynchronize(stream); return fail(RV_ERR_CUDA, std::string("host->device copy: ") + cudaGetErrorString(e)); }
        base = static_cast<const uint8_t*>(d_data.p) + (b0 & 15) - b0;
    }
    try {
        st = decode_on_device(s, base, static_cast<const int64_t*>(d_off.p), n, num_chunks, hints, stream, device, out, r0);
    } catch (const std::exception& e) {
        st = fail(RV_ERR_INVALID, e.what());
    }
    if (st) { const std::string keep = t_error; cudaStreamSynchronize(stream); (void)cudaGetLastError(); t_error = keep; return st; }
    if (n > 0 && h2d_ms) {
        cudaEvent_t* ev = nullptr;
        float t = 0;
        if (t_events.get(device, &ev) == cudaSuccess && cudaEventElapsedTime(&t, ev[4], ev[5]) == cudaSuccess) *h2d_ms += t;
        (void)cudaGetLastError();
    }
    st = arena_to_host(**out, *(*out)->arenas[0], stream, d2h_ms);
    if (st) { rv_result_free(*out); *out = nullptr; }
    return st;
}

bool pipeline_enabled() {
    const char* e = std::getenv("RV_PIPELINE");
    return !(e && e[0] == '0');
}

class WorkerPool {
  public:
    explicit WorkerPool(int device, int n) : device_(device) {
        for (int w = 0; w < n; ++w) std::thread([this, w] { run(w); }).detach();
    }
    void submit(std::function<void(cudaStream_t)> fn) {
        { std::lock_guard<std::mutex> g(mu_); q_.push_back(std::move(fn)); }
        cv_.notify_one();
    }

  private:
    void run(int w) {
        cudaSetDevice(device_);
        bind_thread_to_gpu_node(device_);
        cudaStream_t stream = worker_stream(device_, w);
        for (;;) {
            std::function<void(cudaStream_t)> fn;
            {
                std::unique_lock<std::mutex> g(mu_);
                cv_.wait(g, [&] { return !q_.empty(); });
                fn = std::move(q_.front());
                q_.pop_front();
            }
            fn(stream);
        }
    }
    int device_;
    std::mutex mu_;
    std::condition_variable cv_;
    std::deque<std::function<void(cudaStream_t)>> q_;
};

int worker_count() {
    int want = 4;
    if (const char* ev = std::getenv("RV_WORKERS")) want = std::max(1, std::atoi(ev));
    return std::min(want, 16);
}

WorkerPool& worker_pool(int device) {
    static std::mutex mu;
    static std::map<int, WorkerPool*> pools;
    std::lock_guard<std::mutex> g(mu);
    auto it = pools.find(device);
    if (it != pools.end()) return *it->second;
    WorkerPool* p = new WorkerPool(device, worker_count());
    pools[device] = p;
    return *p;
}

}


struct rv_gather {
    rv_schema* schema = nullptr;
    GatherPlan plan;
    std::vector<std::shared_ptr<Arena>> arenas;
    ~rv_gather() { if (schema) rv_schema_release(schema); }
};

extern "C" {

int64_t rv_gather_meta_len(const rv_schema* s) { return s && s->has_plan ? gather_meta_len(s->plan) : -1; }

rv_status rv_result_gather_meta(const rv_result* r, int64_t batch, int64_t* out, int64_t cap) {
    if (!r || !out || batch < 0 || batch >= int64_t(r->chunks.size())) return fail(RV_ERR_INVALID, "bad argument");
    if (cap < gather_meta_len(r->schema->plan)) return fail(RV_ERR_INVALID, "meta buffer too small");
    gather_meta_of(r->schema->plan, r->chunks[size_t(batch)], out);
    return RV_OK;
}

rv_status rv_gather_plan(const rv_schema* s, const int64_t* metas, int world, rv_gather** out) {
    if (!s || !s->has_plan || !metas || world < 1 || !out) return fail(RV_ERR_INVALID, "bad argument");
    try {
        auto g = std::make_unique<rv_gather>();
        g->schema = rv_schema_retain(const_cast<rv_schema*>(s));
        g->plan = plan_gather(s->plan, metas, world);
        g->arenas.resize(g->plan.groups.size());
        *out = g.release();
        return RV_OK;
    } catch (const std::exception& e) {
        return fail(RV_ERR_OVERFLOW, e.what());
    }
}

int rv_gather_num_groups(const rv_gather* g) { return g ? int(g->plan.groups.size()) : 0; }
int rv_gather_group_of_rank(const rv_gather* g, int rank) {
    return g && rank >= 0 && rank < int(g->plan.group_of_rank.size()) ? g->plan.group_of_rank[size_t(rank)] : -1;
}

rv_status rv_gather_group_info(const rv_gather* g, int group, int64_t* out) {
    if (!g || !out || group < 0 || group >= int(g->plan.groups.size())) return fail(RV_ERR_INVALID, "bad argument");
    const GatherGroup& gg = g->plan.groups[size_t(group)];
    out[0] = gg.first_rank; out[1] = gg.n_ranks; out[2] = int64_t(gg.arena_bytes); out[3] = gg.out.rows;
    int64_t remote = 0;
    for (size_t m = 1; m < gg.jobs.size(); ++m)
        for (const GatherJob& j : gg.jobs[m]) remote += j.kind == GK_RAW ? j.count : (j.kind == GK_OFFSETS ? 4 * j.count : (j.count + 7) / 8);
    out[4] = remote;
    return RV_OK;
}

rv_status rv_gather_alloc(rv_gather* g, int group, void* cuda_stream, void** out_ptr) {
    if (!g || !out_ptr || group < 0 || group >= int(g->plan.groups.size())) return fail(RV_ERR_INVALID, "bad argument");
    int device = 0;
    rv_status st = ensure_cuda(&device);
    if (st) return st;
    auto a = std::make_shared<Arena>();
    a->device = device;
    a->bytes = g->plan.groups[size_t(group)].arena_bytes;
    a->dev = devmem().get(std::max<size_t>(a->bytes, 64), device, &a->dev_actual);
    if (!a->dev) return fail(RV_ERR_CUDA, "device allocation of the gathered arena failed (" + std::to_string(a->bytes) + " bytes)");
    cudaStream_t stream = static_cast<cudaStream_t>(cuda_stream);
    RV_CUDA(cudaMemsetAsync(a->dev, 0, std::max<size_t>(a->bytes, 64), stream));
    RV_CUDA(cudaStreamSynchronize(stream));
    g->arenas[size_t(group)] = a;
    *out_ptr = a->dev;
    return RV_OK;
}

rv_status rv_gather_push(rv_gather* g, int group, int rank, rv_result* mine, int64_t batch, void* dst_base, void* cuda_stream) {
    if (!g || !mine || !dst_base || group < 0 || group >= int(g->plan.groups.size())) return fail(RV_ERR_INVALID, "bad argument");
    const GatherGroup& gg = g->plan.groups[size_t(group)];
    const int m = rank - gg.first_rank;
    if (m < 0 || m >= gg.n_ranks || batch < 0 || batch >= int64_t(mine->chunks.size())) return fail(RV_ERR_INVALID, "rank / batch outside the group");
    Arena& a = *mine->arenas[size_t(batch)];
    if (!a.dev) return fail(RV_ERR_INVALID, "the shard's batch must be device-resident");
    const ChunkOut& c = mine->chunks[size_t(batch)];
    const std::vector<GatherJob>& jobs = gg.jobs[size_t(m)];
    if (jobs.empty()) return RV_OK;
    std::vector<PushJob> pj(jobs.size());
    int64_t bytes = 0;
    for (size_t i = 0; i < jobs.size(); ++i) {
        const GatherJob& j = jobs[i];
        pj[i] = PushJob{static_cast<const uint8_t*>(a.dev) + c.slot_off[size_t(j.slot)], static_cast<uint8_t*>(dst_base) + j.dst_off, j.count, j.param, j.kind, 0};
        bytes += j.kind == GK_RAW ? j.count : (j.kind == GK_OFFSETS ? 4 * j.count : j.count / 8);
    }
    cudaStream_t stream = static_cast<cudaStream_t>(cuda_stream);
    DevBuf d_jobs;
    RV_CUDA(d_jobs.alloc(pj.size() * sizeof(PushJob), stream));
    SyncOnExit guard{stream};
    uint8_t* h = t_scratch.get(pj.size() * sizeof(PushJob));
    if (!h) return fail(RV_ERR_CUDA, "pinned allocation failed");
    std::memcpy(h, pj.data(), pj.size() * sizeof(PushJob));
    RV_CUDA(cudaMemcpyAsync(d_jobs.p, h, pj.size() * sizeof(PushJob), cudaMemcpyHostToDevice, stream));
    const int parts = int(std::max<int64_t>(1, std::min<int64_t>(128, (bytes / int64_t(pj.size())) >> 16)));
    launch_gather_push(static_cast<const PushJob*>(d_jobs.p), int(pj.size()), parts, stream);
    RV_CUDA(cudaGetLastError());
    RV_CUDA(cudaStreamSynchronize(stream));
    guard.armed = false;
    t_launches = 1;
    return RV_OK;
}

rv_status rv_gather_finish(rv_gather* g, int group, rv_result** out) {
    if (!g || !out || group < 0 || group >= int(g->plan.groups.size())) return fail(RV_ERR_INVALID, "bad argument");
    if (!g->arenas[size_t(group)]) return fail(RV_ERR_INVALID, "rv_gather_alloc was not called for this group on this rank");
    auto res = std::make_unique<rv_result>();
    res->schema = rv_schema_retain(g->schema);
    res->chunks.push_back(g->plan.groups[size_t(group)].out);
    res->arenas.push_back(g->arenas[size_t(group)]);
    res->arrow_bytes = exported_bytes(g->schema->plan, res->chunks);
    g->arenas[size_t(group)].reset();
    *out = res.release();
    return RV_OK;
}

void rv_gather_free(rv_gather* g) { delete g; }

rv_status rv_ipc_export(void* dev_ptr, uint8_t* handle64) {
    if (!dev_ptr || !handle64) return fail(RV_ERR_INVALID, "bad argument");
    static_assert(sizeof(cudaIpcMemHandle_t) == 64, "handle size");
    cudaIpcMemHandle_t h;
    RV_CUDA(cudaIpcGetMemHandle(&h, dev_ptr));
    std::memcpy(handle64, &h, 64);
    return RV_OK;
}
rv_status rv_ipc_open(const uint8_t* handle64, void** out) {
    if (!handle64 || !out) return fail(RV_ERR_INVALID, "bad argument");
    cudaIpcMemHandle_t h;
    std::memcpy(&h, handle64, 64);
    RV_CUDA(cudaIpcOpenMemHandle(out, h, cudaIpcMemLazyEnablePeerAccess));
    return RV_OK;
}
rv_status rv_ipc_close(void* p) {
    if (!p) return RV_OK;
    RV_CUDA(cudaIpcCloseMemHandle(p));
    return RV_OK;
}

}


namespace {

rv_status decode_ocf(const uint8_t* file, int64_t len, int64_t num_chunks, const char* const* columns, int64_t n_columns,
                     rv_schema** schema_out, rv_result** out) {
    if (!file || len < 0 || !schema_out || !out) return fail(RV_ERR_INVALID, "null argument");
    *schema_out = nullptr;
    *out = nullptr;
    OcfIndex ix;
    try {
        ix = ocf_index(file, len);
    } catch (const std::exception& e) {
        return fail(RV_ERR_FRAME, e.what());
    }
    rv_schema* s = nullptr;
    rv_status st = rv_schema_parse(ix.schema_json.data(), ix.schema_json.size(), &s);
    if (st) return st;
    if (columns) {
        rv_schema* full = s;
        st = rv_schema_project(full, columns, n_columns, &s);
        rv_schema_release(full);
        if (st) return st;
    }
    struct Release { rv_schema* s; bool armed = true; ~Release() { if (armed) rv_schema_release(s); } } rel{s};
    st = check_decodable(s);
    if (st) return st;
    int device = 0;
    st = ensure_cuda(&device);
    if (st) return st;
    cudaStream_t stream = nullptr;
    const int64_t n = ix.n_records;
    DevBuf d_file, d_blocks, d_off, d_err;
    RV_CUDA(d_file.alloc(size_t(len) + 64, stream));
    RV_CUDA(d_off.alloc(size_t(n + 1) * 8, stream));
    RV_CUDA(d_err.alloc(16, stream));
    SyncOnExit guard{stream};
    RV_CUDA(upload(static_cast<uint8_t*>(d_file.p), file, size_t(len), device, stream));
    if (n > 0) {
        DevicePlan dp;
        st = device_plan(s, device, &dp);
        if (st) return st;
        std::vector<OcfBlockDev> blocks(ix.blocks.size());
        for (size_t i = 0; i < blocks.size(); ++i) blocks[i] = OcfBlockDev{ix.blocks[i].data_off, ix.blocks[i].size, ix.blocks[i].count, ix.blocks[i].rec_base};
        RV_CUDA(d_blocks.alloc(blocks.size() * sizeof(OcfBlockDev), stream));
        RV_CUDA(cudaMemcpyAsync(d_blocks.p, blocks.data(), blocks.size() * sizeof(OcfBlockDev), cudaMemcpyHostToDevice, stream));
        RV_CUDA(cudaMemsetAsync(d_err.p, 0xFF, 8, stream));
        OcfParams q{};
        q.data = static_cast<const uint8_t*>(d_file.p);
        q.blocks = static_cast<const OcfBlockDev*>(d_blocks.p);
        q.n_blocks = int32_t(blocks.size());
        q.nodes = dp.nodes; q.n_nodes = int32_t(s->plan.nodes.size());
        q.sym_off = dp.sym_off; q.sym_bytes = dp.sym_bytes;
        q.offsets = static_cast<int64_t*>(d_off.p);
        q.n_records = n;
        q.end_off = ix.end_off;
        q.err = static_cast<unsigned long long*>(d_err.p);
        launch_ocf_offsets(q, stream);
        RV_CUDA(cudaGetLastError());
        unsigned long long err_word = ~0ull;
        RV_CUDA(cudaMemcpyAsync(&err_word, d_err.p, 8, cudaMemcpyDeviceToHost, stream));
        RV_CUDA(cudaStreamSynchronize(stream));
        if (err_word != ~0ull) {
            const uint32_t code = uint32_t(err_word & 0xFF);
            return fail(rv_status(code), std::string(err_text(code)) + " (record " + std::to_string(int64_t(err_word >> 8)) + ")");
        }
    }
    try {
        st = decode_on_device(s, static_cast<const uint8_t*>(d_file.p), static_cast<const int64_t*>(d_off.p), n, num_chunks, InputHints{}, stream, device, out);
    } catch (const std::exception& e) {
        st = fail(RV_ERR_INVALID, e.what());
    }
    if (st) return st;
    float ms = 0;
    st = arena_to_host(**out, *(*out)->arenas[0], stream, &ms);
    if (st) { rv_result_free(*out); *out = nullptr; return st; }
    guard.armed = false;
    rel.armed = false;
    *schema_out = s;
    return RV_OK;
}

}

extern "C" rv_status rv_decode_ocf_host(const uint8_t* file, int64_t len, int64_t num_chunks, rv_schema** schema_out, rv_result** out) {
    return decode_ocf(file, len, num_chunks, nullptr, 0, schema_out, out);
}

extern "C" rv_status rv_decode_ocf_host_projected(const uint8_t* file, int64_t len, int64_t num_chunks, const char* const* columns,
                                                  int64_t n_columns, rv_schema** schema_out, rv_result** out) {
    if (!columns && n_columns != 0) return fail(RV_ERR_INVALID, "null argument");
    if (!columns) return fail(RV_ERR_INVALID, "column projection: the column list is empty");
    return decode_ocf(file, len, num_chunks, columns, n_columns, schema_out, out);
}

extern "C" {

rv_status rv_result_to_host(rv_result* r) {
    if (!r) return fail(RV_ERR_INVALID, "null result");
    float ms = 0;
    for (auto& a : r->arenas) {
        rv_status st = arena_to_host(*r, *a, nullptr, &ms);
        if (st) return st;
    }
    t_timings[5] = ms;
    return RV_OK;
}

rv_status rv_decode_host(const rv_schema* s_, const uint8_t* data, const int64_t* offsets, int64_t n,
                         int64_t num_chunks, rv_result** out) {
    return rv_decode_host_framed(s_, data, offsets, n, num_chunks, nullptr, out);
}

rv_status rv_decode_host_framed(const rv_schema* s_, const uint8_t* data, const int64_t* offsets, int64_t n,
                                int64_t num_chunks, const rv_framing* framing_, rv_result** out) {
    if (!out) return fail(RV_ERR_INVALID, "null argument");
    *out = nullptr;
    rv_schema* s = const_cast<rv_schema*>(s_);
    rv_status st = check_decodable(s);
    if (st) return st;
    st = framing_ok(framing_);
    if (st) return st;
    const rv_framing framing = framing_ ? *framing_ : rv_framing{0, 0, -1};
    if (n < 0 || (n > 0 && (!data || !offsets))) return fail(RV_ERR_INVALID, "bad input pointers");
    int device = 0;
    st = ensure_cuda(&device);
    if (st) return st;
    const int64_t k = clamp_chunks(num_chunks, n);
    float h2d = 0, d2h = 0;
    if (k < 2 || n / k < 16384 || !pipeline_enabled()) {
        st = decode_host_range(s, data, offsets, 0, n, num_chunks, nullptr, device, out, &h2d, &d2h, framing);
        t_timings[4] = h2d;
        t_timings[5] = d2h;
        return st;
    }
    const int64_t chunk_rows = n / k;
    struct Call {
        std::mutex mu;
        std::condition_variable cv;
        int64_t left;
        float acc[6] = {0, 0, 0, 0, 0, 0};
        int launches = 0, passes = 0;
        long long slow = 0;
        const char* walker = "none";
    } call;
    call.left = k;
    std::vector<rv_result*> parts(size_t(k), nullptr);
    std::vector<rv_status> status(size_t(k), RV_OK);
    std::vector<std::string> message{size_t(k), std::string()};
    WorkerPool& pool = worker_pool(device);
    for (int64_t i = 0; i < k; ++i) {
        pool.submit([&, i](cudaStream_t stream) {
            const int64_t r0 = i * chunk_rows, r1 = (i == k - 1) ? n : r0 + chunk_rows;
            float hm = 0, dm = 0;
            rv_status rc;
            try {
                rc = decode_host_range(s, data, offsets, r0, r1, 1, stream, device, &parts[size_t(i)], &hm, &dm, framing);
            } catch (const std::exception& e) {
                rc = fail(RV_ERR_INVALID, e.what());
            }
            status[size_t(i)] = rc;
            if (rc) message[size_t(i)] = t_error;
            std::lock_guard<std::mutex> g(call.mu);
            for (int q = 0; q < 4; ++q) call.acc[q] += t_timings[q];
            call.acc[4] += hm;
            call.acc[5] += dm;
            call.launches += t_launches;
            call.passes = std::max(call.passes, t_passes);
            call.slow += t_slow_tiles;
            call.walker = t_walker;
            if (--call.left == 0) call.cv.notify_all();
        });
    }
    {
        std::unique_lock<std::mutex> g(call.mu);
        call.cv.wait(g, [&] { return call.left == 0; });
    }
    for (int q = 0; q < 6; ++q) t_timings[q] = call.acc[q];
    t_launches = call.launches;
    t_passes = call.passes;
    t_slow_tiles = call.slow;
    t_walker = call.walker;
    auto res = std::make_unique<rv_result>();
    res->schema = rv_schema_retain(s);
    rv_status first = RV_OK;
    for (int64_t i = 0; i < k; ++i) {
        if (status[size_t(i)] && !first) { first = status[size_t(i)]; t_error = message[size_t(i)]; }
    }
    for (int64_t i = 0; i < k; ++i) {
        rv_result* part = parts[size_t(i)];
        if (!part) continue;
        if (!first) {
            res->chunks.push_back(std::move(part->chunks[0]));
            res->arenas.push_back(part->arenas[0]);
            res->arrow_bytes += part->arrow_bytes;
        }
        rv_result_free(part);
    }
    if (first) return first;
    *out = res.release();
    return RV_OK;
}

int64_t rv_result_num_batches(const rv_result* r) { return r ? int64_t(r->chunks.size()) : 0; }
int64_t rv_result_num_rows(const rv_result* r, int64_t batch) {
    if (!r || batch < 0 || batch >= int64_t(r->chunks.size())) return -1;
    return r->chunks[size_t(batch)].rows;
}
int64_t rv_result_arrow_bytes(const rv_result* r) { return r ? r->arrow_bytes : 0; }
int64_t rv_result_buffer_bytes(const rv_result* r) {
    if (!r) return 0;
    int64_t total = 0;
    const Arena* last = nullptr;
    for (auto& a : r->arenas) {
        if (a.get() != last) total += int64_t(a->host ? a->host_bytes : a->bytes);
        last = a.get();
    }
    return total;
}

rv_status rv_result_export(rv_result* r, int64_t batch, struct ArrowArray* out_array, struct ArrowSchema* out_schema) {
    if (!r || !out_array) return fail(RV_ERR_INVALID, "null argument");
    if (batch < 0 || batch >= int64_t(r->chunks.size())) return fail(RV_ERR_INVALID, "batch index out of range");
    if (!r->arenas[size_t(batch)]->host) return fail(RV_ERR_INVALID, "result is device-resident: call rv_result_to_host() or rv_result_export_device()");
    if (out_schema) {
        rv_status st = rv_schema_export_arrow(r->schema, out_schema);
        if (st) return st;
    }
    export_batch(r->schema->plan, r->chunks[size_t(batch)], static_cast<const uint8_t*>(r->arenas[size_t(batch)]->host), r->arenas[size_t(batch)], out_array);
    return RV_OK;
}

rv_status rv_result_export_device(rv_result* r, int64_t batch, struct ArrowDeviceArray* out_array, struct ArrowSchema* out_schema) {
    if (!r || !out_array) return fail(RV_ERR_INVALID, "null argument");
    if (batch < 0 || batch >= int64_t(r->chunks.size())) return fail(RV_ERR_INVALID, "batch index out of range");
    if (!r->arenas[size_t(batch)]->dev) return fail(RV_ERR_INVALID, "result was moved to host memory: use rv_result_export()");
    if (out_schema) {
        rv_status st = rv_schema_export_arrow(r->schema, out_schema);
        if (st) return st;
    }
    export_batch(r->schema->plan, r->chunks[size_t(batch)], static_cast<const uint8_t*>(r->arenas[size_t(batch)]->dev), r->arenas[size_t(batch)], &out_array->array);
    out_array->device_id = r->arenas[size_t(batch)]->device;
    out_array->device_type = ARROW_DEVICE_CUDA;
    out_array->sync_event = nullptr;
    out_array->reserved[0] = out_array->reserved[1] = out_array->reserved[2] = 0;
    return RV_OK;
}

void rv_result_free(rv_result* r) { delete r; }

void* rv_host_alloc(size_t bytes) {
    size_t actual = 0;
    void* p = pinned().get(bytes, &actual);
    if (!p) {
        t_error = "cudaHostAlloc failed (no CUDA device, or out of pinnable memory)";
        return nullptr;
    }
    std::lock_guard<std::mutex> g(g_host_mu);
    g_host_sizes[p] = actual;
    return p;
}
void rv_host_free(void* p) {
    if (!p) return;
    size_t actual = 0;
    {
        std::lock_guard<std::mutex> g(g_host_mu);
        auto it = g_host_sizes.find(p);
        if (it == g_host_sizes.end()) return;
        actual = it->second;
        g_host_sizes.erase(it);
    }
    pinned().put(p, actual);
}

int rv_last_timings(float* out_ms, int cap) {
    int n = cap < 6 ? cap : 6;
    for (int i = 0; i < n; ++i) out_ms[i] = t_timings[i];
    return n;
}
int rv_last_launch_count(void) { return t_launches; }
int rv_last_passes(void) { return t_passes; }
rv_status rv_dev_rebase_i32(int32_t* d_dst, const int32_t* d_src, int64_t n, int32_t add, void* cuda_stream) {
    if (n < 0 || (n > 0 && (!d_dst || !d_src))) return fail(RV_ERR_INVALID, "bad argument");
    launch_rebase_i32(d_dst, d_src, n, add, static_cast<cudaStream_t>(cuda_stream));
    RV_CUDA(cudaGetLastError());
    return RV_OK;
}

rv_status rv_dev_concat_bits(uint32_t* d_dst_words, int64_t dst_bit, const uint32_t* d_src_words, int64_t nbits, void* cuda_stream) {
    if (nbits < 0 || dst_bit < 0 || (nbits > 0 && (!d_dst_words || !d_src_words))) return fail(RV_ERR_INVALID, "bad argument");
    launch_concat_bits(d_dst_words, dst_bit, d_src_words, nbits, static_cast<cudaStream_t>(cuda_stream));
    RV_CUDA(cudaGetLastError());
    return RV_OK;
}

void* rv_internal_dev_get(size_t bytes, int device, size_t* actual) { return devmem().get(bytes, device, actual); }
void rv_internal_dev_put(void* p, size_t actual, int device) { devmem().put(p, actual, device); }
const void* rv_schema_avro_root(const rv_schema* s) { return s ? s->avro.get() : nullptr; }
int rv_schema_is_projection(const rv_schema* s) { return s && !s->keep.empty() ? 1 : 0; }
void rv_set_last_error(const char* msg) { t_error = msg ? msg : ""; }

const char* rv_last_walker(void) { return t_walker; }
const char* rv_schema_jit_status(const rv_schema* s) {
    if (!s) return "null schema";
    std::lock_guard<std::mutex> g(const_cast<rv_schema*>(s)->mu);
    int device = 0;
    if (cudaGetDevice(&device) != cudaSuccess) (void)cudaGetLastError();
    auto it = s->jit.find(device);
    t_error = (it != s->jit.end() && it->second.tried) ? it->second.status : "not attempted yet";
    return t_error.c_str();
}
long long rv_last_slow_tiles(void) { return t_slow_tiles; }
void rv_set_jit_enabled(int enabled) { g_jit_override.store(enabled < 0 ? -1 : (enabled ? 1 : 0)); }
void rv_schema_forget_stats(const rv_schema* s_) {
    rv_schema* s = const_cast<rv_schema*>(s_);
    if (!s) return;
    std::lock_guard<std::mutex> g(s->mu);
    s->stats = SchemaStats();
}

int64_t rv_schema_walker_source(const rv_schema* s, char* buf, size_t cap) {
    if (!s || !s->has_plan) return -1;
    const std::string src = generate_walker_source(s->plan);
    if (buf && cap) {
        const size_t n = std::min(cap - 1, src.size());
        std::memcpy(buf, src.data(), n);
        buf[n] = 0;
    }
    return int64_t(src.size());
}

rv_status rv_schema_precompile(const rv_schema* s, const char* arch) {
    rv_status st = check_decodable(s);
    if (st) return st;
    std::vector<char> cubin;
    std::string log;
    if (!jit_cubin(generate_kernel_source(s->plan), arch && *arch ? arch : "sm_90a", &cubin, &log, false)) return fail(RV_ERR_CUDA, "NVRTC: " + log);
    return RV_OK;
}
const char* rv_last_error(void) { return t_error.c_str(); }
const char* rv_version(void) { return "pyruhvro_b200 0.2.0 (sm_90a)"; }

}
```

### pyruhvro_b200/csrc/jit.cpp

```cpp
#include "jit.hpp"

#include <dlfcn.h>
#include <sys/stat.h>
#include <unistd.h>

#include <cstdio>
#include <cstdlib>
#include <cstring>
#include <fstream>
#include <mutex>
#include <algorithm>
#include <atomic>
#include <sstream>

namespace rv {

extern const char* const kHdrDevTypes;
extern const char* const kHdrDevCore;
extern const char* const kHdrDevKernels;

namespace {

struct Gen {
    const Plan& p;
    std::ostringstream fns;
    int unchecked = 0;
    int n_ilists = 0;
    int n_skip_runs = 0;

    void top(std::ostringstream& body) {
        const int n = int(p.nodes.size());
        for (int pc = 0; pc < n;) {
            if (!(p.nodes[size_t(pc)].flags & NF_SKIP)) {
                node(body, pc, 0, "vtop", 2);
                pc = p.nodes[size_t(pc)].end;
                continue;
            }
            const int r = n_skip_runs++;
            body << ind(2) << "// fields outside the column projection: the FAST emit resumes where the count walk left them\n";
            body << ind(2) << "if (MODE == WM_EMIT && C::kShared) {\n";
            body << ind(3) << "c.pos = q.skip_end[" << r << "];\n";
            body << ind(2) << "} else {\n";
            for (; pc < n && (p.nodes[size_t(pc)].flags & NF_SKIP); pc = p.nodes[size_t(pc)].end) node(body, pc, 0, "vtop", 3);
            body << ind(3) << "if (MODE == WM_COUNT) q.skip_end[" << r << "] = c.pos;\n";
            body << ind(2) << "}\n";
        }
    }

    void skip(std::ostringstream& o, int pc, int D, const std::string& parent, int in) {
        const DNode& nd = p.nodes[size_t(pc)];
        const std::string v = "v" + std::to_string(pc);
        budget(o, nd, in);
        if (nd.kind == NK_UNION) {
            o << ind(in) << "const int s" << pc << " = op_union<WM_COUNT, 0>(c, " << parent << ", " << nd.aux << ", -1, 0u);\n";
            int k = 0;
            for (int ch = pc + 1; ch < nd.end; ch = p.nodes[size_t(ch)].end, ++k)
                node(o, ch, D, "(s" + std::to_string(pc) + " == " + std::to_string(k) + ")", in);
            return;
        }
        o << ind(in) << "bool " << v << " = " << parent << ";\n";
        if (nd.flags & NF_NULLABLE)
            o << ind(in) << "if (" << v << ") " << v << " = rd_branch<MODE == WM_COUNT>(c, " << ((nd.flags & NF_NULL_FIRST) ? "true" : "false") << ");\n";
        switch (nd.kind) {
            case NK_REC:
                for (int ch = pc + 1; ch < nd.end; ch = p.nodes[size_t(ch)].end) node(o, ch, D, v, in);
                break;
            case NK_LIST:
            case NK_MAP: {
                std::ostringstream f;
                f << "template <int MODE, class C>\nRV_HD void item_" << pc << "(C& c) {\n";
                f << ind(1) << "const bool vtop = true;\n";
                const int outer_unchecked = unchecked;
                unchecked = 20;
                for (int ch = pc + 1; ch < nd.end; ch = p.nodes[size_t(ch)].end) node(f, ch, D + 1, "vtop", 1);
                unchecked = outer_unchecked + 20;
                f << "}\n\n";
                fns << f.str();
                o << ind(in) << "if (" << v << ") {\n";
                o << ind(in + 1) << "int64_t rem = 0;\n";
                o << ind(in + 1) << "for (;;) {\n";
                o << ind(in + 2) << "if (rem == 0) {\n";
                o << ind(in + 3) << "const int b = skip_block(c, rem, " << ((nd.flags & NF_ZERO_ITEMS) ? "true" : "false") << ");\n";
                o << ind(in + 3) << "if (b == 0) break;\n";
                o << ind(in + 3) << "if (b == 2) continue;\n";
                o << ind(in + 2) << "}\n";
                o << ind(in + 2) << "item_" << pc << "<MODE>(c);\n";
                o << ind(in + 2) << "--rem;\n";
                o << ind(in + 2) << "if (item_stop<WM_COUNT>(c)) break;\n";
                o << ind(in + 1) << "}\n";
                o << ind(in) << "}\n";
                break;
            }
            default:
                o << ind(in) << "skip_leaf(c, " << v << ", " << int(nd.kind) << ", " << (nd.kind == NK_ENUM ? nd.aux2 : nd.aux) << ");\n";
                break;
        }
    }

    void items_par(int pc, int L) {
        const DNode& nd = p.nodes[size_t(pc)];
        std::vector<int> inner;
        for (int i = pc + 1; i < nd.end; ++i)
            if (p.nodes[size_t(i)].stream >= 0) inner.push_back(p.nodes[size_t(i)].stream);
        std::ostringstream& f = fns;
        f << "template <class C>\nRV_HD void items_par_" << pc << "(C& c, const uint32_t l0, const uint32_t n, Cur& q) {\n";
        f << ind(1) << "const uint32_t tl = c.row0 % uint32_t(kBlock), lane = tl % 32u;\n";
        f << ind(1) << "const uint32_t incl = warp_scan_incl(n, lane), excl = incl - n;  // the lane's items are flat [excl, incl)\n";
        f << ind(1) << "const uint32_t tot = warp_shfl(incl, 31u, lane);\n";
        f << ind(1) << "const uint32_t row_base = warp_shfl(q.v[" << nd.stream << "], 0u, lane);\n";
        for (int s : inner) {
            f << ind(1) << "const uint32_t b" << s << " = warp_shfl(q.v[" << s << "], 0u, lane);\n";
            f << ind(1) << "uint32_t carry" << s << " = 0;\n";
        }
        f << ind(1) << "const uint32_t end_saved = c.end;\n";
        f << ind(1) << "c.end = 0xFFFFFFFFu;  // items of other lanes' records: validated by the count walk\n";
        f << ind(1) << "for (uint32_t r = 0; r < tot; r += 32u) {\n";
        f << ind(2) << "const uint32_t fi = r + lane;\n";
        f << ind(2) << "const bool act = fi < tot;\n";
        f << ind(2) << "uint32_t o = 0, eo = 0;  // owner lane: the last lane whose first item is <= fi\n";
        f << ind(2) << "for (uint32_t b = 16u; b; b >>= 1) {\n";
        f << ind(3) << "const uint32_t e = warp_shfl(excl, o + b, lane);\n";
        f << ind(3) << "if (e <= fi) { o += b; eo = e; }\n";
        f << ind(2) << "}\n";
        f << ind(2) << "const uint32_t ol0 = warp_shfl(l0, o, lane);  // where the owner's list starts\n";
        f << ind(2) << "const uint32_t p0 = act ? ol0 + itab_get(c, (" << L << " * kItemEntries + (fi - eo)) * kBlock + (tl & ~31u) + o) : c.pos;\n";
        f << ind(2) << "Cur m;\n";
        for (int s : inner) f << ind(2) << "m.v[" << s << "] = 0;\n";
        f << ind(2) << "c.pos = p0;\n";
        f << ind(2) << "if (act) item_" << pc << "<WM_COUNT>(c, row_base + fi, m);  // the item's share of every inner stream\n";
        for (int s : inner) {
            f << ind(2) << "{\n";
            f << ind(3) << "const uint32_t x = warp_scan_incl(m.v[" << s << "], lane);\n";
            f << ind(3) << "m.v[" << s << "] = b" << s << " + carry" << s << " + x - m.v[" << s << "];\n";
            f << ind(3) << "carry" << s << " += warp_shfl(x, 31u, lane);\n";
            f << ind(2) << "}\n";
        }
        f << ind(2) << "c.pos = p0;\n";
        f << ind(2) << "if (act) item_" << pc << "<WM_EMIT>(c, row_base + fi, m);\n";
        f << ind(1) << "}\n";
        f << ind(1) << "c.end = end_saved;\n";
        f << ind(1) << "// the lane's cursors after its own items = the next lane's before them\n";
        for (int s : inner) {
            f << ind(1) << "{\n";
            f << ind(2) << "const uint32_t nx = warp_shfl(q.v[" << s << "], (lane + 1u) & 31u, lane);\n";
            f << ind(2) << "q.v[" << s << "] = lane == 31u ? b" << s << " + carry" << s << " : nx;\n";
            f << ind(1) << "}\n";
        }
        f << ind(1) << "c.pos = l0 + itab_get(c, (" << L << " * kItemEntries + kItemSlots) * kBlock + tl);\n";
        f << ind(1) << "(void)row_base;\n";
        f << "}\n\n";
    }

    static int worst_bytes(const DNode& nd) {
        int b = (nd.flags & NF_NULLABLE) ? 10 : 0;
        switch (nd.kind) {
            case NK_BOOL: return b + 1;
            case NK_F32: return b + 4;
            case NK_F64: return b + 8;
            case NK_NULL: case NK_REC: return b;
            case NK_FIXED: return b;
            case NK_DEC_FIXED: return b + 16;
            case NK_LIST: case NK_MAP: return b + 20;
            default: return b + 10;
        }
    }
    void budget(std::ostringstream& o, const DNode& nd, int in) {
        const int w = worst_bytes(nd);
        if (unchecked + w > int(kWindowPad) - 16) {
            o << ind(in) << "eof_check<MODE>(c);\n";
            unchecked = 0;
        }
        unchecked += w;
    }

    static std::string ind(int n) { return std::string(size_t(n) * 4, ' '); }

    static const char* kind_name(int k) {
        static const char* names[] = {"int32", "int64", "float", "double", "bool", "string", "enum", "null", "record", "union", "list", "map",
                                      "bytes", "fixed", "decimal(bytes)", "decimal(fixed)", "uuid"};
        return names[k];
    }

    void node(std::ostringstream& o, int pc, int D, const std::string& parent, int in) {
        const DNode& nd = p.nodes[size_t(pc)];
        const std::string v = "v" + std::to_string(pc);
        const int sv = (nd.flags & NF_VALIDITY) ? int(nd.slot_v) : -1;
        const std::string md = "<MODE, " + std::to_string(D) + ">";
        o << ind(in) << "// node " << pc << ": " << kind_name(nd.kind) << ((nd.flags & NF_NULLABLE) ? " (nullable)" : "")
          << ((nd.flags & NF_SKIP) ? " (skipped)" : "") << "\n";
        if (nd.kind == NK_NULL) return;
        if (nd.flags & NF_SKIP) return skip(o, pc, D, parent, in);
        budget(o, nd, in);
        if (nd.kind == NK_UNION) {
            o << ind(in) << "const int s" << pc << " = op_union" << md << "(c, " << parent << ", " << nd.aux << ", " << nd.slot_a << ", row);\n";
            int k = 0;
            for (int ch = pc + 1; ch < nd.end; ch = p.nodes[size_t(ch)].end, ++k)
                node(o, ch, D, "(s" + std::to_string(pc) + " == " + std::to_string(k) + ")", in);
            return;
        }
        o << ind(in) << "bool " << v << " = " << parent << ";\n";
        if (nd.flags & NF_NULLABLE)
            o << ind(in) << "if (" << v << ") " << v << " = rd_branch<MODE == WM_COUNT>(c, " << ((nd.flags & NF_NULL_FIRST) ? "true" : "false") << ");\n";
        switch (nd.kind) {
            case NK_I32: o << ind(in) << "op_i32" << md << "(c, " << v << ", " << nd.slot_a << ", " << sv << ", row);\n"; break;
            case NK_I64: o << ind(in) << "op_i64" << md << "(c, " << v << ", " << nd.slot_a << ", " << sv << ", row);\n"; break;
            case NK_F32: o << ind(in) << "op_f32" << md << "(c, " << v << ", " << nd.slot_a << ", " << sv << ", row);\n"; break;
            case NK_F64: o << ind(in) << "op_f64" << md << "(c, " << v << ", " << nd.slot_a << ", " << sv << ", row);\n"; break;
            case NK_BOOL: o << ind(in) << "op_bool" << md << "(c, " << v << ", " << nd.slot_a << ", " << sv << ", row);\n"; break;
            case NK_STR:
                o << ind(in) << "op_str" << md << "(c, " << v << ", " << nd.slot_a << ", " << nd.slot_b << ", " << sv << ", " << nd.stream << ", row, q.v[" << nd.stream << "]);\n";
                break;
            case NK_BYTES:
                o << ind(in) << "op_str" << md << "(c, " << v << ", " << nd.slot_a << ", " << nd.slot_b << ", " << sv << ", " << nd.stream << ", row, q.v[" << nd.stream << "]);\n";
                break;
            case NK_FIXED: o << ind(in) << "op_fixed" << md << "(c, " << v << ", " << nd.aux << ", " << nd.slot_a << ", " << sv << ", row);\n"; break;
            case NK_UUID: o << ind(in) << "op_uuid" << md << "(c, " << v << ", " << nd.slot_a << ", " << sv << ", row);\n"; break;
            case NK_DEC_BYTES: o << ind(in) << "op_decimal" << md << "(c, " << v << ", -1, " << nd.slot_a << ", " << sv << ", row);\n"; break;
            case NK_DEC_FIXED: o << ind(in) << "op_decimal" << md << "(c, " << v << ", " << nd.aux << ", " << nd.slot_a << ", " << sv << ", row);\n"; break;
            case NK_ENUM:
                o << ind(in) << "op_enum" << md << "(c, " << v << ", " << nd.slot_a << ", " << nd.slot_b << ", " << sv << ", " << nd.stream << ", row, "
                  << nd.aux << ", " << nd.aux2 << ", q.v[" << nd.stream << "]);\n";
                break;
            case NK_REC:
                if (sv >= 0) o << ind(in) << "if (MODE == WM_EMIT) put_bit<" << D << ">(c, " << sv << ", row, " << v << ");\n";
                for (int ch = pc + 1; ch < nd.end; ch = p.nodes[size_t(ch)].end) node(o, ch, D, v, in);
                break;
            case NK_LIST:
            case NK_MAP: {
                std::ostringstream f;
                f << "template <int MODE, class C>\nRV_HD void item_" << pc << "(C& c, const uint32_t row, Cur& q) {\n";
                f << ind(1) << "const bool vtop = true;\n";
                const int outer_unchecked = unchecked;
                unchecked = 20;
                for (int ch = pc + 1; ch < nd.end; ch = p.nodes[size_t(ch)].end) node(f, ch, D + 1, "vtop", 1);
                unchecked = outer_unchecked + 20;
                f << "}\n\n";
                fns << f.str();
                const bool par = D == 0 && !(nd.flags & NF_ZERO_ITEMS);
                const int L = par ? n_ilists++ : -1;
                if (par) items_par(pc, L);
                const std::string ent = "(" + std::to_string(L) + " * kItemEntries + ";
                o << ind(in) << "{\n";
                o << ind(in + 1) << "const uint32_t first = (MODE == WM_EMIT) ? q.v[" << nd.stream << "] : 0u;\n";
                o << ind(in + 1) << "uint32_t total = 0;\n";
                o << ind(in + 1) << "bool seq = true;\n";
                if (par) o << ind(in + 1) << "const uint32_t l0 = c.pos;  // where the list starts\n";
                if (par) {
                    o << "#if !defined(RV_ABL_SEQITEMS)\n";
                    o << ind(in + 1) << "if constexpr (MODE == WM_EMIT && C::kShared) if (item_parallel_on()) {  // (warp-uniform)\n";
                    o << ind(in + 2) << "const uint32_t n = itab_get(c, " << ent << "kItemSlots + 1) * kBlock + tl);\n";
                    o << ind(in + 2) << "seq = warp_any(n > uint32_t(kItemSlots), tl % 32u);\n";
                    o << ind(in + 2) << "if (!seq) { total = n; items_par_" << pc << "(c, l0, n, q); }\n";
                    o << ind(in + 1) << "}\n";
                    o << "#endif\n";
                }
                o << ind(in + 1) << "if (seq && " << v << ") {\n";
                o << ind(in + 2) << "int64_t rem = 0;\n";
                o << ind(in + 2) << "for (;;) {\n";
                o << ind(in + 3) << "if (rem == 0) {\n";
                o << ind(in + 4) << "const int b = rd_block<MODE == WM_COUNT>(c, rem, total, " << ((nd.flags & NF_ZERO_ITEMS) ? "true" : "false") << ");\n";
                o << ind(in + 4) << "if (b == 0) break;\n";
                o << ind(in + 4) << "if (b == 2) continue;\n";
                o << ind(in + 3) << "}\n";
                if (par) {
                    o << "#if !defined(RV_ABL_SEQITEMS)\n";
                    o << ind(in + 3) << "if (MODE == WM_COUNT && C::kShared && total < uint32_t(kItemSlots) && item_parallel_on()) itab_put(c, " << ent << "total) * kBlock + tl, c.pos - l0);\n";
                    o << "#endif\n";
                }
                o << ind(in + 3) << "item_" << pc << "<MODE>(c, first + total, q);\n";
                o << ind(in + 3) << "++total;\n";
                o << ind(in + 3) << "--rem;\n";
                o << ind(in + 3) << "if (item_stop<MODE>(c)) break;\n";
                o << ind(in + 2) << "}\n";
                o << ind(in + 1) << "}\n";
                if (par) {
                    o << "#if !defined(RV_ABL_SEQITEMS)\n";
                    o << ind(in + 1) << "if (MODE == WM_COUNT && C::kShared && item_parallel_on()) {  // where the list ends, and how many items it has\n";
                    o << ind(in + 2) << "const uint32_t e = c.pos - l0;\n";
                    o << ind(in + 2) << "itab_put(c, " << ent << "kItemSlots) * kBlock + tl, e);\n";
                    o << ind(in + 2) << "itab_put(c, " << ent << "kItemSlots + 1) * kBlock + tl, (total > uint32_t(kItemSlots) || e > 0xFFu) ? kItemSeq : total);\n";
                    o << ind(in + 1) << "}\n";
                    o << "#endif\n";
                }
                o << ind(in + 1) << "(void)seq;\n";
                o << ind(in + 1) << "list_finish" << md << "(c, " << v << ", first, total, " << nd.slot_a << ", " << sv << ", q.v[" << nd.stream << "], row);\n";
                o << ind(in) << "}\n";
                break;
            }
            default: break;
        }
    }
};

uint64_t fnv1a(const std::string& s, uint64_t h = 1469598103934665603ull) {
    for (unsigned char ch : s) { h ^= ch; h *= 1099511628211ull; }
    return h;
}

typedef struct _nvrtcProgram* nvrtcProgram;
struct Nvrtc {
    void* h = nullptr;
    int (*CreateProgram)(nvrtcProgram*, const char*, const char*, int, const char* const*, const char* const*) = nullptr;
    int (*CompileProgram)(nvrtcProgram, int, const char* const*) = nullptr;
    int (*GetCUBINSize)(nvrtcProgram, size_t*) = nullptr;
    int (*GetCUBIN)(nvrtcProgram, char*) = nullptr;
    int (*GetProgramLogSize)(nvrtcProgram, size_t*) = nullptr;
    int (*GetProgramLog)(nvrtcProgram, char*) = nullptr;
    int (*DestroyProgram)(nvrtcProgram*) = nullptr;
    std::string err;
};

Nvrtc& nvrtc() {
    static Nvrtc n;
    static std::once_flag once;
    std::call_once(once, [] {
        const char* cands[] = {std::getenv("RV_NVRTC_LIB"), "libnvrtc.so.12", "/usr/local/cuda/lib64/libnvrtc.so.12", "libnvrtc.so",
                               "/usr/local/cuda/lib64/libnvrtc.so"};
        for (const char* c : cands) {
            if (!c || !*c) continue;
            n.h = dlopen(c, RTLD_NOW | RTLD_LOCAL);
            if (n.h) break;
        }
        if (!n.h) { n.err = "libnvrtc.so.12 not found (set RV_NVRTC_LIB)"; return; }
        auto sym = [&](const char* name) { void* p = dlsym(n.h, name); if (!p) n.err = std::string("missing NVRTC symbol ") + name; return p; };
        n.CreateProgram = reinterpret_cast<decltype(n.CreateProgram)>(sym("nvrtcCreateProgram"));
        n.CompileProgram = reinterpret_cast<decltype(n.CompileProgram)>(sym("nvrtcCompileProgram"));
        n.GetCUBINSize = reinterpret_cast<decltype(n.GetCUBINSize)>(sym("nvrtcGetCUBINSize"));
        n.GetCUBIN = reinterpret_cast<decltype(n.GetCUBIN)>(sym("nvrtcGetCUBIN"));
        n.GetProgramLogSize = reinterpret_cast<decltype(n.GetProgramLogSize)>(sym("nvrtcGetProgramLogSize"));
        n.GetProgramLog = reinterpret_cast<decltype(n.GetProgramLog)>(sym("nvrtcGetProgramLog"));
        n.DestroyProgram = reinterpret_cast<decltype(n.DestroyProgram)>(sym("nvrtcDestroyProgram"));
    });
    return n;
}

std::string cache_dir() {
    if (const char* e = std::getenv("RV_JIT_CACHE")) return e;
    Dl_info info;
    if (dladdr(reinterpret_cast<const void*>(&cache_dir), &info) && info.dli_fname) {
        std::string path = info.dli_fname;
        size_t slash = path.rfind('/');
        if (slash != std::string::npos) return path.substr(0, slash) + "/_jitcache";
    }
    return "/tmp/pyruhvro_b200_jitcache-" + std::to_string(static_cast<long long>(getuid()));
}

bool cache_dir_ok(const std::string& dir) {
    mkdir(dir.c_str(), 0700);
    struct stat st;
    if (stat(dir.c_str(), &st) != 0 || !S_ISDIR(st.st_mode)) return false;
    return st.st_uid == getuid() && (st.st_mode & (S_IWGRP | S_IWOTH)) == 0;
}

}

std::string generate_walker_source(const Plan& plan) {
    Gen g{plan, {}};
    std::ostringstream body;
    g.top(body);
    std::ostringstream o;
    o << "// generated by pyruhvro_b200 jit.cpp from the decode plan — do not edit\n";
    o << "#include \"dev_core.cuh\"\n\nnamespace rv {\nnamespace gen {\n\n";
    o << "// per-lane cursors (one per stream) live in registers: every index below is a literal\n";
    o << "struct Cur { uint32_t v[" << std::max<size_t>(1, plan.streams.size()) << "];";
    if (g.n_skip_runs) o << " uint32_t skip_end[" << g.n_skip_runs << "];";
    o << " };\n\n";
    o << g.fns.str();
    o << "struct Walker {\n";
    o << "    static constexpr bool kRegCursors = true;\n";
    o << "    static constexpr int kStreams = " << plan.streams.size() << ";\n";
    o << "    static constexpr uint32_t kItemBytes = " << item_table_bytes(g.n_ilists) << ";  // " << g.n_ilists << " item-parallel lists\n";
    o << "    using Cur = rv::gen::Cur;\n";
    o << "    template <int MODE, class C>\n    static RV_HD void walk(C& c, int, Cur& q) {\n";
    o << "        const uint32_t row = c.row0;\n        const bool vtop = c.in_range;\n";
    if (g.n_ilists) o << "        const uint32_t tl = c.row0 % uint32_t(kBlock);  // lane in tile\n        (void)tl;\n";
    o << body.str();
    o << "        eof_check<MODE>(c);\n";
    o << "    }\n";
    o << "    template <class C>\n    static RV_HD void zero_offsets(C& c, int tid) {\n";
    int i = 0;
    for (const DNode& nd : plan.nodes)
        if (!(nd.flags & NF_SKIP) && (nd.kind == NK_STR || nd.kind == NK_ENUM || nd.kind == NK_LIST || nd.kind == NK_MAP || nd.kind == NK_BYTES))
            o << "        if (tid == " << (i++ % 32) << ") static_cast<int32_t*>(buf_ptr(c, " << nd.slot_a << "))[0] = 0;\n";
    o << "        (void)c; (void)tid;\n    }\n};\n\n}  // namespace gen\n}  // namespace rv\n";
    return o.str();
}

int item_parallel_lists(const Plan& plan) {
    Gen g{plan, {}};
    std::ostringstream body;
    g.top(body);
    return g.n_ilists;
}

static int env_int(const char* name, int dflt) {
    const char* v = std::getenv(name);
    return v && *v ? std::atoi(v) : dflt;
}

std::string generate_kernel_source(const Plan& plan) {
    std::ostringstream o;
    const int minb = env_int("RV_JIT_MINB", 3);
    if (const char* defs = std::getenv("RV_JIT_DEFS")) {
        std::string d(defs), item;
        std::istringstream is(d);
        while (std::getline(is, item, ';')) {
            if (item.empty()) continue;
            const size_t eq = item.find('=');
            o << "#define " << item.substr(0, eq) << " " << (eq == std::string::npos ? "1" : item.substr(eq + 1)) << "\n";
        }
    }
    o << "#define RV_KBLOCK " << kBlock << "\n";
    o << "#include \"dev_kernels.cuh\"\n";
    o << generate_walker_source(plan);
    o << "\nextern \"C\" __global__ void __launch_bounds__(rv::kBlock, " << minb
      << ") rvj_fused(const rv::DecodeParams p) { rv::fused_body<rv::gen::Walker>(p, int(blockIdx.x)); }\n";
    return o.str();
}

bool jit_cubin(const std::string& source, const std::string& arch, std::vector<char>* cubin, std::string* log, bool ignore_cache) {
    uint64_t h = fnv1a(source);
    h = fnv1a(kHdrDevTypes, h);
    h = fnv1a(kHdrDevCore, h);
    h = fnv1a(kHdrDevKernels, h);
    h = fnv1a(arch, h);
    char name[64];
    std::snprintf(name, sizeof name, "/%016llx.cubin", static_cast<unsigned long long>(h));
    const std::string dir = cache_dir(), path = dir + name;
    const bool use_cache = !(std::getenv("RV_JIT_NO_CACHE") && *std::getenv("RV_JIT_NO_CACHE") == '1') && cache_dir_ok(dir);
    if (use_cache && !ignore_cache) {
        std::ifstream f(path, std::ios::binary);
        if (f) {
            cubin->assign(std::istreambuf_iterator<char>(f), std::istreambuf_iterator<char>());
            if (!cubin->empty()) return true;
        }
    }
    Nvrtc& n = nvrtc();
    if (!n.h || !n.err.empty()) {
        if (log) *log = "NVRTC unavailable: " + n.err;
        return false;
    }
    nvrtcProgram prog = nullptr;
    const char* hdr_src[] = {kHdrDevTypes, kHdrDevCore, kHdrDevKernels};
    const char* hdr_names[] = {"dev_types.h", "dev_core.cuh", "dev_kernels.cuh"};
    if (n.CreateProgram(&prog, source.c_str(), "rv_walker.cu", 3, hdr_src, hdr_names) != 0) {
        if (log) *log = "nvrtcCreateProgram failed";
        return false;
    }
    const std::string arch_opt = "--gpu-architecture=" + arch;
    const char* opts[] = {arch_opt.c_str(), "-std=c++17", "-lineinfo"};
    const int rc = n.CompileProgram(prog, 3, opts);
    size_t ls = 0;
    n.GetProgramLogSize(prog, &ls);
    std::string l(ls, '\0');
    if (ls > 1) n.GetProgramLog(prog, &l[0]);
    if (log) *log = l;
    if (rc != 0) {
        n.DestroyProgram(&prog);
        return false;
    }
    size_t cs = 0;
    n.GetCUBINSize(prog, &cs);
    cubin->resize(cs);
    n.GetCUBIN(prog, cubin->data());
    n.DestroyProgram(&prog);
    if (use_cache && cs) {
        static std::atomic<unsigned> seq{0};
        const std::string tmp = path + ".tmp" + std::to_string(static_cast<long long>(getpid())) + "." + std::to_string(seq.fetch_add(1));
        std::ofstream f(tmp, std::ios::binary);
        if (f) {
            f.write(cubin->data(), std::streamsize(cs));
            f.close();
            if (!f || std::rename(tmp.c_str(), path.c_str()) != 0) std::remove(tmp.c_str());
        }
    }
    return true;
}

}
```

### pyruhvro_b200/csrc/jit.hpp

```cpp
#pragma once
#include <string>
#include <vector>

#include "plan.hpp"

namespace rv {

std::string generate_walker_source(const Plan& plan);

int item_parallel_lists(const Plan& plan);

std::string generate_kernel_source(const Plan& plan);

bool jit_cubin(const std::string& source, const std::string& arch, std::vector<char>* cubin, std::string* log, bool ignore_cache = false);

}
```

Measured before the change: 3.915 billion.

## Add wide 384-row tile JIT walker for schemas with many streams

For schemas with more than eight streams, the decoder now JIT-compiles a second walker whose block and tile size is 384 rows. It keeps separate per-tile JIT state, rescales the collected span and UTF-8 statistics to the new tile, and computes the host span hint per tile. Larger tiles amortize per-tile fixed costs such as cursor setup and prefetch over more rows. In exchange each tile needs more shared memory for cursors and staging, so fewer CTAs fit per SM (capped at two), and there is an extra NVRTC compile.

```diff
diff --git a/include/ruhvro_b200.h b/include/ruhvro_b200.h
--- a/include/ruhvro_b200.h
+++ b/include/ruhvro_b200.h
@@ -112,11 +112,14 @@
 void rv_schema_forget_stats(const rv_schema* s);
 
 const char* rv_last_walker(void);
+int rv_last_tile(void);
+int rv_schema_max_tile(const rv_schema* s);
 const char* rv_schema_jit_status(const rv_schema* s);
 long long rv_last_slow_tiles(void);
 void rv_set_jit_enabled(int enabled);
 
 int64_t rv_schema_walker_source(const rv_schema* s, char* buf, size_t cap);
+int64_t rv_schema_kernel_source(const rv_schema* s, int tile, char* buf, size_t cap);
 
 rv_status rv_schema_precompile(const rv_schema* s, const char* arch);
 
diff --git a/pyruhvro_b200/__init__.py b/pyruhvro_b200/__init__.py
--- a/pyruhvro_b200/__init__.py
+++ b/pyruhvro_b200/__init__.py
@@ -89,6 +89,11 @@
     L.rv_schema_forget_stats.argtypes = [vp]
     L.rv_schema_forget_stats.restype = None
     L.rv_last_walker.restype = cp
+    L.rv_last_tile.restype = ctypes.c_int
+    L.rv_schema_max_tile.restype = ctypes.c_int
+    L.rv_schema_max_tile.argtypes = [vp]
+    L.rv_schema_kernel_source.restype = i64
+    L.rv_schema_kernel_source.argtypes = [vp, ctypes.c_int, cp, ctypes.c_size_t]
     L.rv_set_jit_enabled.argtypes = [ctypes.c_int]
     L.rv_set_jit_enabled.restype = None
     L.rv_schema_walker_source.restype = i64
diff --git a/pyruhvro_b200/csrc/dev_kernels.cuh b/pyruhvro_b200/csrc/dev_kernels.cuh
--- a/pyruhvro_b200/csrc/dev_kernels.cuh
+++ b/pyruhvro_b200/csrc/dev_kernels.cuh
@@ -140,7 +140,7 @@
     const int64_t ft = int64_t(tile_id) + p.prefetch_dist;
     if (p.prefetch_dist > 0 && ft < p.n_tiles) {
         const Tile f = tile_of(p, int(ft));
-        if (tid < 17 && f.r0 + 16 * tid <= p.n) l2_prefetch_line(p.offsets + f.r0 + 16 * tid);
+        if (tid <= kBlock / 16 && f.r0 + 16 * tid <= p.n) l2_prefetch_line(p.offsets + f.r0 + 16 * tid);
         if (tid == kPrefetchLane) {
             w.f0 = __ldg(p.offsets + f.r0);
             w.f1 = __ldg(p.offsets + f.r0 + f.nrec);
diff --git a/pyruhvro_b200/csrc/dev_types.h b/pyruhvro_b200/csrc/dev_types.h
--- a/pyruhvro_b200/csrc/dev_types.h
+++ b/pyruhvro_b200/csrc/dev_types.h
@@ -91,6 +91,8 @@
 constexpr int kBlock = RV_KBLOCK;
 static_assert(kBlock % 32 == 0 && kBlock >= 64 && kBlock <= 1024, "tiles are whole warps");
 constexpr int kWarps = kBlock / 32;
+constexpr int kWideTile = 384;
+constexpr int kWideStreams = 8;
 
 enum CtrlWord : int {
     CW_ERR = 0,
@@ -140,7 +142,7 @@
 #if defined(__CUDACC__)
 __host__ __device__
 #endif
-constexpr uint32_t item_table_bytes(int n_lists) { return uint32_t(n_lists) * uint32_t(kItemEntries) * uint32_t(kBlock); }
+constexpr uint32_t item_table_bytes(int n_lists, int tile = kBlock) { return uint32_t(n_lists) * uint32_t(kItemEntries) * uint32_t(tile); }
 
 struct SmemMap {
     uint32_t nodes, ttot, tbase, adj, flags, mbar, ptrs, items, cur, in, stage, total;
@@ -149,7 +151,8 @@
 #if defined(__CUDACC__)
 __host__ __device__
 #endif
-inline SmemMap smem_map(int n_nodes, int n_streams, int n_slots, uint32_t data_cap, uint32_t stage_cap, bool alias_cur, uint32_t item_bytes) {
+inline SmemMap smem_map(int n_nodes, int n_streams, int n_slots, uint32_t data_cap, uint32_t stage_cap, bool alias_cur, uint32_t item_bytes,
+                        int tile = kBlock) {
     SmemMap m;
     m.nodes = 0;
     m.ttot = uint32_t(n_nodes) * 32u;
@@ -160,7 +163,7 @@
     m.ptrs = m.mbar + 16u;
     m.items = (m.ptrs + uint32_t(n_slots) * 8u + 15u) & ~15u;
     m.cur = (m.items + item_bytes + 15u) & ~15u;
-    const uint32_t cur_bytes = uint32_t(n_streams) * kBlock * 4u;
+    const uint32_t cur_bytes = uint32_t(n_streams) * uint32_t(tile) * 4u;
     m.in = alias_cur ? m.cur : ((m.cur + cur_bytes + 15u) & ~15u);
     m.stage = (m.in + data_cap + kWindowPad + 15u) & ~15u;
     if (alias_cur) {
diff --git a/pyruhvro_b200/csrc/engine.cu b/pyruhvro_b200/csrc/engine.cu
--- a/pyruhvro_b200/csrc/engine.cu
+++ b/pyruhvro_b200/csrc/engine.cu
@@ -6,6 +6,7 @@
 #include <algorithm>
 #include <atomic>
 #include <chrono>
+#include <cmath>
 #include <condition_variable>
 #include <cstdio>
 #include <cstring>
@@ -37,6 +38,7 @@
 thread_local float t_timings[6] = {0, 0, 0, 0, 0, 0};
 thread_local int t_launches = 0;
 thread_local const char* t_walker = "none";
+thread_local int t_tile = 0;
 thread_local long long t_slow_tiles = 0;
 thread_local int t_passes = 0;
 
@@ -336,7 +338,26 @@
     double in_per_row = 0;
     unsigned long long max_span = 0;
     unsigned long long max_utf8 = 0;
+    int tile = 0;
 };
+
+static SchemaStats stats_at(const SchemaStats& st, int tile, const Plan& plan) {
+    if (!st.valid || st.tile == tile || st.tile == 0) return st;
+    SchemaStats o = st;
+    o.tile = tile;
+    const double g = std::sqrt(double(tile) / double(st.tile));
+    auto carry = [&](unsigned long long mx, double per_row, double fixed) -> unsigned long long {
+        if (!mx) return 0;
+        const double excess = std::max(0.0, double(mx) - (per_row * st.tile + fixed));
+        return static_cast<unsigned long long>(std::ceil(per_row * tile + fixed + excess * g));
+    };
+    double utf8_per_row = 0, n_utf8 = 0;
+    for (size_t i = 0; i < plan.streams.size() && i < st.per_row.size(); ++i)
+        if (!plan.streams[i].is_rows) { utf8_per_row += st.per_row[i]; n_utf8 += 1; }
+    o.max_span = carry(st.max_span, st.in_per_row, 0.0);
+    o.max_utf8 = carry(st.max_utf8, utf8_per_row, 31.0 * n_utf8);
+    return o;
+}
 
 struct rv_schema {
     std::atomic<int> refs{1};
@@ -350,7 +371,7 @@
     bool has_plan = false;
     std::mutex mu;
     std::map<int, DevicePlan> dev;
-    std::map<int, JitState> jit;
+    std::map<std::pair<int, int>, JitState> jit;
     SchemaStats stats;
 };
 
@@ -394,13 +415,13 @@
     return "sm_" + std::to_string(prop.major) + std::to_string(prop.minor) + ((prop.major >= 9) ? "a" : "");
 }
 
-JitState ensure_jit(rv_schema* s, int device) {
+JitState ensure_jit(rv_schema* s, int device, int tile) {
     if (!jit_enabled()) { JitState d; d.tried = true; d.status = "disabled (RV_JIT=0 / rv_set_jit_enabled(0))"; return d; }
     std::lock_guard<std::mutex> g(s->mu);
-    JitState& j = s->jit[device];
+    JitState& j = s->jit[{device, tile}];
     if (j.tried) return j;
     j.tried = true;
-    const std::string source = generate_kernel_source(s->plan), arch = device_arch(device);
+    const std::string source = generate_kernel_source(s->plan, tile), arch = device_arch(device);
     for (int attempt = 0; attempt < 2; ++attempt) {
         std::vector<char> cubin;
         std::string log;
@@ -564,9 +585,19 @@
 
 struct InputHints {
     int64_t total_bytes = -1;
-    int64_t max_span = -1;
+    const int64_t* offsets = nullptr;
     rv_framing framing = {0, 0, -1};
 };
+
+int64_t max_tile_span(const int64_t* offsets, int64_t n, int64_t k, int tile) {
+    const int64_t cr = n / k;
+    int64_t mx = 0;
+    for (int64_t j = 0; j < k; ++j) {
+        const int64_t cs = j * cr, ce = (j == k - 1) ? n : cs + cr;
+        for (int64_t a = cs; a < ce; a += tile) mx = std::max(mx, offsets[std::min(a + tile, ce)] - offsets[a]);
+    }
+    return mx;
+}
 
 rv_status decode_on_device(rv_schema* s, const uint8_t* d_data, const int64_t* d_offsets, int64_t n, int64_t num_chunks,
                            const InputHints& hints, cudaStream_t stream, int device, rv_result** out, int64_t record_base = 0) {
@@ -617,16 +648,6 @@
     DevicePlan dp;
     rv_status st = device_plan(s, device, &dp);
     if (st) return st;
-    const int64_t tpc = std::max<int64_t>(1, (chunk_rows + kBlock - 1) / kBlock);
-    const int64_t tiles_last = (last_rows + kBlock - 1) / kBlock;
-    const int64_t n_tiles = tpc * (k - 1) + tiles_last;
-    if (n_tiles > 0x7FFFFFF0ll) return fail(RV_ERR_INVALID, "too many records for one call");
-
-    const JitState jit = ensure_jit(s, device);
-    const bool use_jit = jit.ok;
-    t_walker = use_jit ? "jit" : "interp";
-    const int plan_nodes = use_jit ? 0 : int(plan.nodes.size());
-
     SchemaStats stats;
     {
         std::lock_guard<std::mutex> g(s->mu);
@@ -635,8 +656,7 @@
 
     DecodeParams p{};
     p.data = d_data; p.offsets = d_offsets; p.n = n; p.chunk_rows = chunk_rows; p.k = k;
-    p.tiles_per_chunk = int32_t(tpc); p.n_tiles = int32_t(n_tiles);
-    p.nodes = dp.nodes; p.n_nodes = int32_t(plan_nodes); p.n_streams = S; p.n_slots = n_slots;
+    p.n_streams = S; p.n_slots = n_slots;
     p.sym_off = dp.sym_off; p.sym_bytes = dp.sym_bytes; p.stream_slot = dp.stream_slot;
     p.n_utf8 = 0;
     for (int i = 0; i < S; ++i) p.n_utf8 += plan.streams[size_t(i)].is_rows ? 0 : 1;
@@ -645,16 +665,29 @@
     p.frame_id = uint32_t(hints.framing.schema_id >= 0 ? hints.framing.schema_id : 0);
 
     const size_t limit = 227 * 1024;
-    const size_t cur_bytes = size_t(S) * kBlock * 4;
-    const uint32_t item_bytes = use_jit ? item_table_bytes(item_parallel_lists(plan)) : 0u;
-    const size_t fixed = smem_map(plan_nodes, S, n_slots, 0, 0, use_jit, item_bytes).stage;
-    if (fixed + (use_jit ? cur_bytes : 0) + 2048 > limit) return fail(RV_ERR_SCHEMA, "schema too wide for the shared-memory cursor table");
+    int tile = kBlock;
+    bool use_jit = false;
+    int plan_nodes = 0;
+    uint32_t item_bytes = 0;
+    size_t cur_bytes = 0, fixed = 0;
+    int64_t span_hint = -1;
+    auto set_walker = [&](int tile_, bool jit_) {
+        tile = tile_;
+        use_jit = jit_;
+        plan_nodes = use_jit ? 0 : int(plan.nodes.size());
+        cur_bytes = size_t(S) * size_t(tile) * 4;
+        item_bytes = use_jit ? item_table_bytes(item_parallel_lists(plan), tile) : 0u;
+        fixed = smem_map(plan_nodes, S, n_slots, 0, 0, use_jit, item_bytes, tile).stage;
+        span_hint = hints.offsets ? max_tile_span(hints.offsets, n, k, tile) : -1;
+    };
+    auto too_wide = [&] { return fixed + (use_jit ? cur_bytes : 0) + 2048 > limit; };
+    auto ctas_per_sm = [&](size_t bytes) { const size_t c = (228 * 1024) / (bytes + 1024); return tile > kBlock ? std::min<size_t>(c, 2) : c; };
     size_t smem_bytes = 0;
     auto configure = [&](const SchemaStats& st_) {
         const double in_per_row = hints.total_bytes >= 0 ? double(hints.total_bytes) / double(n) : (st_.in_per_row > 0 ? st_.in_per_row : 128.0);
-        unsigned long long max_span = hints.max_span >= 0 ? static_cast<unsigned long long>(hints.max_span)
-                                      : (st_.max_span ? st_.max_span + st_.max_span / 16 : static_cast<unsigned long long>(in_per_row * kBlock * 1.25));
-        size_t want_in = std::min<size_t>(size_t(max_span), size_t(in_per_row * kBlock * env_double("RV_IN_CLAMP", 1.5))) + 48;
+        unsigned long long max_span = span_hint >= 0 ? static_cast<unsigned long long>(span_hint)
+                                      : (st_.max_span ? st_.max_span + st_.max_span / 16 : static_cast<unsigned long long>(in_per_row * tile * 1.25));
+        size_t want_in = std::min<size_t>(size_t(max_span), size_t(in_per_row * tile * env_double("RV_IN_CLAMP", 1.5))) + 48;
         want_in = std::max<size_t>(align_up(want_in, 64), 2048);
         const size_t room = (limit - fixed - 64) & ~size_t(15);
         const size_t min_stage = use_jit ? align_up(cur_bytes, 16) : 0;
@@ -665,14 +698,14 @@
             double utf8_per_row = 0;
             if (st_.valid) for (int i = 0; i < S; ++i) if (!plan.streams[size_t(i)].is_rows) utf8_per_row += st_.per_row[size_t(i)];
             size_t want_out = seen;
-            if (st_.valid) want_out = std::min<size_t>(seen, size_t(utf8_per_row * kBlock * env_double("RV_OUT_CLAMP", 1.5)) + size_t(p.n_utf8) * 31);
+            if (st_.valid) want_out = std::min<size_t>(seen, size_t(utf8_per_row * tile * env_double("RV_OUT_CLAMP", 1.5)) + size_t(p.n_utf8) * 31);
             cap_stage = align_up(want_out + 64, 64);
             if (const char* ev_ = std::getenv("RV_NO_STAGE_OUT")) if (ev_[0] == '1') cap_stage = 0;
         }
         cap_stage = std::max(cap_stage, min_stage);
         if (cap_in + cap_stage > room) cap_stage = std::max<size_t>(min_stage, (room - cap_in) & ~size_t(15));
-        if (hints.max_span < 0 && (st_.max_span || st_.max_utf8)) {
-            auto ctas = [&](size_t in_b, size_t st_b) { return (228 * 1024) / (smem_map(plan_nodes, S, n_slots, uint32_t(in_b), uint32_t(st_b), use_jit, item_bytes).total + 1024); };
+        if (span_hint < 0 && (st_.max_span || st_.max_utf8)) {
+            auto ctas = [&](size_t in_b, size_t st_b) { return ctas_per_sm(smem_map(plan_nodes, S, n_slots, uint32_t(in_b), uint32_t(st_b), use_jit, item_bytes, tile).total); };
             const size_t floor_in = st_.max_span ? std::min(cap_in, std::max<size_t>(align_up(size_t(st_.max_span) + 48, 64), 2048)) : cap_in;
             const size_t floor_stage = st_.max_utf8 ? std::min(cap_stage, std::max(min_stage, size_t(align_up(size_t(st_.max_utf8) + 64, 64)))) : cap_stage;
             const size_t want = ctas(cap_in, cap_stage) + 1;
@@ -686,15 +719,45 @@
         p.smem_data_cap = uint32_t(cap_in);
         p.smem_stage_cap = uint32_t(cap_stage);
         const size_t pad_smem = size_t(env_double("RV_SMEM_PAD", 0));
-        smem_bytes = std::min<size_t>(smem_map(plan_nodes, S, n_slots, p.smem_data_cap, p.smem_stage_cap, use_jit, item_bytes).total + pad_smem, limit);
+        smem_bytes = std::min<size_t>(smem_map(plan_nodes, S, n_slots, p.smem_data_cap, p.smem_stage_cap, use_jit, item_bytes, tile).total + pad_smem, limit);
         p.prefetch_dist = 0;
         if (!(std::getenv("RV_NO_PREFETCH") && std::getenv("RV_NO_PREFETCH")[0] == '1')) {
-            const int ctas_per_sm = int(std::max<size_t>(1, std::min<size_t>(8, (228 * 1024) / (smem_bytes + 1024))));
+            const int ctas = int(std::max<size_t>(1, std::min<size_t>(8, ctas_per_sm(smem_bytes))));
             int sms = 132;
             cudaDeviceGetAttribute(&sms, cudaDevAttrMultiProcessorCount, device);
-            p.prefetch_dist = sms * ctas_per_sm;
+            p.prefetch_dist = sms * ctas;
         }
     };
+    auto choose_tile = [&]() -> JitState {
+        const char* ev_ = std::getenv("RV_TILE");
+        if (S > kWideStreams && jit_enabled() && !(ev_ && std::atoi(ev_) == kBlock)) {
+            set_walker(kWideTile, true);
+            if (!too_wide()) {
+                const SchemaStats st_ = stats_at(stats, kWideTile, plan);
+                configure(st_);
+                const size_t need = st_.valid ? smem_bytes
+                                              : smem_map(0, S, n_slots, p.smem_data_cap, uint32_t(align_up(cur_bytes, 16)), true, item_bytes, tile).total;
+                if (ctas_per_sm(need) >= 2) {
+                    const JitState j = ensure_jit(s, device, kWideTile);
+                    if (j.ok) return j;
+                }
+            }
+        }
+        const JitState j = ensure_jit(s, device, kBlock);
+        set_walker(kBlock, j.ok);
+        return j;
+    };
+    const JitState jit = choose_tile();
+    t_walker = use_jit ? "jit" : "interp";
+    t_tile = tile;
+    if (too_wide()) return fail(RV_ERR_SCHEMA, "schema too wide for the shared-memory cursor table");
+
+    const int64_t tpc = std::max<int64_t>(1, (chunk_rows + tile - 1) / tile);
+    const int64_t tiles_last = (last_rows + tile - 1) / tile;
+    const int64_t n_tiles = tpc * (k - 1) + tiles_last;
+    if (n_tiles > 0x7FFFFFF0ll) return fail(RV_ERR_INVALID, "too many records for one call");
+    p.tiles_per_chunk = int32_t(tpc); p.n_tiles = int32_t(n_tiles);
+    p.nodes = dp.nodes; p.n_nodes = int32_t(plan_nodes);
 
     const int nv = int(plan.validity_slots.size());
     const size_t ctrl_words = size_t(CW_CHUNK_TOT) + chunk_tot.size();
@@ -745,9 +808,9 @@
 
     for (int pass = 0; pass < 3; ++pass) {
         ++t_passes;
-        configure(stats);
+        configure(stats_at(stats, tile, plan));
         if (trace)
-            trace_line += "smem=" + std::to_string(smem_bytes) + "(in " + std::to_string(p.smem_data_cap) + " stage " + std::to_string(p.smem_stage_cap) +
+            trace_line += "tile=" + std::to_string(tile) + " smem=" + std::to_string(smem_bytes) + "(in " + std::to_string(p.smem_data_cap) + " stage " + std::to_string(p.smem_stage_cap) +
                           " items " + std::to_string(item_bytes) + "; largest tile seen: span " + std::to_string(stats.max_span) +
                           " utf8 " + std::to_string(stats.max_utf8) + ") ";
         uint8_t* arena = nullptr;
@@ -766,8 +829,8 @@
         std::memset(h_misc, 0, misc_bytes);
         unsigned long long* hc = reinterpret_cast<unsigned long long*>(h_misc + off_ctrl);
         hc[CW_ERR] = ~0ull;
-        hc[CW_MAX_SPAN] = stats.max_span;
-        hc[CW_MAX_UTF8] = stats.max_utf8;
+        hc[CW_MAX_SPAN] = stats.tile == tile ? stats.max_span : 0ull;
+        hc[CW_MAX_UTF8] = stats.tile == tile ? stats.max_utf8 : 0ull;
         if (!count_only) {
             void** hb = reinterpret_cast<void**>(h_misc + off_bufs);
             for (int j = 0; j < k; ++j)
@@ -795,12 +858,12 @@
         RV_CUDA(cudaEventRecord(ev[0], stream));
         if (use_jit) {
             void* args[] = {&p};
-            const cudaError_t le = cudaLaunchKernel(reinterpret_cast<const void*>(jit.fused), dim3(unsigned(p.n_tiles)), dim3(kBlock), args, smem_bytes, stream);
+            const cudaError_t le = cudaLaunchKernel(reinterpret_cast<const void*>(jit.fused), dim3(unsigned(p.n_tiles)), dim3(unsigned(tile)), args, smem_bytes, stream);
             if (le != cudaSuccess) {
                 (void)cudaGetLastError();
                 {
                     std::lock_guard<std::mutex> g(s->mu);
-                    JitState& j = s->jit[device];
+                    JitState& j = s->jit[{device, tile}];
                     j.ok = false;
                     j.status = std::string("launch of the compiled walker was rejected: ") + cudaGetErrorString(le);
                 }
@@ -845,8 +908,10 @@
             }
             if (hints.total_bytes >= 0) ss.in_per_row = double(hints.total_bytes) / double(n);
             else if (hb_ctrl[CW_IN_LAST] >= hb_ctrl[CW_IN_FIRST]) ss.in_per_row = double(hb_ctrl[CW_IN_LAST] - hb_ctrl[CW_IN_FIRST]) / double(n);
+            if (ss.tile != tile) ss.max_span = ss.max_utf8 = 0;
             ss.max_span = std::max(ss.max_span, hb_ctrl[CW_MAX_SPAN]);
             ss.max_utf8 = std::max(ss.max_utf8, hb_ctrl[CW_MAX_UTF8]);
+            ss.tile = tile;
             ss.valid = true;
             stats = ss;
         }
@@ -1111,16 +1176,7 @@
         const int64_t total = offsets[r1] - b0;
         if (total < 0) return fail(RV_ERR_INVALID, "offsets are not monotonic");
         hints.total_bytes = total;
-        {
-            const int64_t k = clamp_chunks(num_chunks, n);
-            const int64_t cr = n / k;
-            int64_t mx = 0;
-            for (int64_t j = 0; j < k; ++j) {
-                const int64_t cs = r0 + j * cr, ce = (j == k - 1) ? r1 : cs + cr;
-                for (int64_t a = cs; a < ce; a += kBlock) mx = std::max(mx, offsets[std::min(a + kBlock, ce)] - offsets[a]);
-            }
-            hints.max_span = mx;
-        }
+        hints.offsets = offsets + r0;
         RV_CUDA(d_data.alloc(size_t(total) + 64, stream));
         RV_CUDA(d_off.alloc(size_t(n + 1) * 8, stream));
         cudaEvent_t* ev = nullptr;
@@ -1487,6 +1543,7 @@
         int launches = 0, passes = 0;
         long long slow = 0;
         const char* walker = "none";
+        int tile = 0;
     } call;
     call.left = k;
     std::vector<rv_result*> parts(size_t(k), nullptr);
@@ -1513,6 +1570,7 @@
             call.passes = std::max(call.passes, t_passes);
             call.slow += t_slow_tiles;
             call.walker = t_walker;
+            call.tile = call.tile ? std::min(call.tile, t_tile) : t_tile;
             if (--call.left == 0) call.cv.notify_all();
         });
     }
@@ -1525,6 +1583,7 @@
     t_passes = call.passes;
     t_slow_tiles = call.slow;
     t_walker = call.walker;
+    t_tile = call.tile;
     auto res = std::make_unique<rv_result>();
     res->schema = rv_schema_retain(s);
     rv_status first = RV_OK;
@@ -1645,12 +1704,18 @@
 void rv_set_last_error(const char* msg) { t_error = msg ? msg : ""; }
 
 const char* rv_last_walker(void) { return t_walker; }
+int rv_last_tile(void) { return t_tile; }
+int rv_schema_max_tile(const rv_schema* s) {
+    if (!s || !s->has_plan) return -1;
+    return int(s->plan.streams.size()) > kWideStreams ? kWideTile : kBlock;
+}
 const char* rv_schema_jit_status(const rv_schema* s) {
     if (!s) return "null schema";
     std::lock_guard<std::mutex> g(const_cast<rv_schema*>(s)->mu);
     int device = 0;
     if (cudaGetDevice(&device) != cudaSuccess) (void)cudaGetLastError();
-    auto it = s->jit.find(device);
+    auto it = s->jit.find({device, kBlock});
+    if (it == s->jit.end() || !it->second.tried) it = s->jit.find({device, kWideTile});
     t_error = (it != s->jit.end() && it->second.tried) ? it->second.status : "not attempted yet";
     return t_error.c_str();
 }
@@ -1674,12 +1739,23 @@
     return int64_t(src.size());
 }
 
+int64_t rv_schema_kernel_source(const rv_schema* s, int tile, char* buf, size_t cap) {
+    if (!s || !s->has_plan || (tile != kBlock && tile != rv_schema_max_tile(s))) return -1;
+    const std::string src = generate_kernel_source(s->plan, tile);
+    if (buf && cap) {
+        const size_t n = std::min(cap - 1, src.size());
+        std::memcpy(buf, src.data(), n);
+        buf[n] = 0;
+    }
+    return int64_t(src.size());
+}
+
 rv_status rv_schema_precompile(const rv_schema* s, const char* arch) {
     rv_status st = check_decodable(s);
     if (st) return st;
     std::vector<char> cubin;
     std::string log;
-    if (!jit_cubin(generate_kernel_source(s->plan), arch && *arch ? arch : "sm_90a", &cubin, &log, false)) return fail(RV_ERR_CUDA, "NVRTC: " + log);
+    if (!jit_cubin(generate_kernel_source(s->plan, rv_schema_max_tile(s)), arch && *arch ? arch : "sm_90a", &cubin, &log, false)) return fail(RV_ERR_CUDA, "NVRTC: " + log);
     return RV_OK;
 }
 const char* rv_last_error(void) { return t_error.c_str(); }
diff --git a/pyruhvro_b200/csrc/jit.cpp b/pyruhvro_b200/csrc/jit.cpp
--- a/pyruhvro_b200/csrc/jit.cpp
+++ b/pyruhvro_b200/csrc/jit.cpp
@@ -354,7 +354,7 @@
 
 }
 
-std::string generate_walker_source(const Plan& plan) {
+std::string generate_walker_source(const Plan& plan, int tile) {
     Gen g{plan, {}};
     std::ostringstream body;
     g.top(body);
@@ -369,7 +369,7 @@
     o << "struct Walker {\n";
     o << "    static constexpr bool kRegCursors = true;\n";
     o << "    static constexpr int kStreams = " << plan.streams.size() << ";\n";
-    o << "    static constexpr uint32_t kItemBytes = " << item_table_bytes(g.n_ilists) << ";  // " << g.n_ilists << " item-parallel lists\n";
+    o << "    static constexpr uint32_t kItemBytes = " << item_table_bytes(g.n_ilists, tile) << ";  // " << g.n_ilists << " item-parallel lists\n";
     o << "    using Cur = rv::gen::Cur;\n";
     o << "    template <int MODE, class C>\n    static RV_HD void walk(C& c, int, Cur& q) {\n";
     o << "        const uint32_t row = c.row0;\n        const bool vtop = c.in_range;\n";
@@ -398,9 +398,9 @@
     return v && *v ? std::atoi(v) : dflt;
 }
 
-std::string generate_kernel_source(const Plan& plan) {
+std::string generate_kernel_source(const Plan& plan, int tile) {
     std::ostringstream o;
-    const int minb = env_int("RV_JIT_MINB", 3);
+    const int minb = env_int("RV_JIT_MINB", tile > kBlock ? 2 : 3);
     if (const char* defs = std::getenv("RV_JIT_DEFS")) {
         std::string d(defs), item;
         std::istringstream is(d);
@@ -410,9 +410,9 @@
             o << "#define " << item.substr(0, eq) << " " << (eq == std::string::npos ? "1" : item.substr(eq + 1)) << "\n";
         }
     }
-    o << "#define RV_KBLOCK " << kBlock << "\n";
+    o << "#define RV_KBLOCK " << tile << "\n";
     o << "#include \"dev_kernels.cuh\"\n";
-    o << generate_walker_source(plan);
+    o << generate_walker_source(plan, tile);
     o << "\nextern \"C\" __global__ void __launch_bounds__(rv::kBlock, " << minb
       << ") rvj_fused(const rv::DecodeParams p) { rv::fused_body<rv::gen::Walker>(p, int(blockIdx.x)); }\n";
     return o.str();
diff --git a/pyruhvro_b200/csrc/jit.hpp b/pyruhvro_b200/csrc/jit.hpp
--- a/pyruhvro_b200/csrc/jit.hpp
+++ b/pyruhvro_b200/csrc/jit.hpp
@@ -6,11 +6,11 @@
 
 namespace rv {
 
-std::string generate_walker_source(const Plan& plan);
+std::string generate_walker_source(const Plan& plan, int tile = kBlock);
 
 int item_parallel_lists(const Plan& plan);
 
-std::string generate_kernel_source(const Plan& plan);
+std::string generate_kernel_source(const Plan& plan, int tile);
 
 bool jit_cubin(const std::string& source, const std::string& arch, std::vector<char>* cubin, std::string* log, bool ignore_cache = false);
 
```

Result: faster. 4.563 billion (median of 6 runs) (+16.5%).
